# imazen/codec-eval

Measured on AMD Instinct MI355X. Metric: metric MP/s (SSIMULACRA2+DSSIM+Butteraugli) at 1/2/4/8 GPU; HBM-roofline %, higher is better.
Workload: dtype f32

## Files before the change

### codec-eval_amd/csrc/ce_api.cpp

```cpp
#include <algorithm>
#include <atomic>
#include <condition_variable>
#include <functional>
#include <mutex>
#include <thread>
#include <cmath>
#include <cstdlib>
#include <cstring>
#include <new>

#include "ce_internal.h"

static thread_local std::string g_err_noctx;

int ce_fail(ce_ctx *ctx, int code, const std::string &msg)
{
    if (ctx) ctx->err = msg; else g_err_noctx = msg;
    return code;
}

int ce_bad_length(ce_ctx *ctx, size_t want, size_t got)
{
    return ce_fail(ctx, CE_ERR_BAD_LENGTH, "Invalid image size: expected " + std::to_string(want) + " bytes, got " + std::to_string(got));
}

int ce_validate_pair(ce_ctx *ctx, size_t ref_len, size_t test_len, size_t w, size_t h)
{
    if (ref_len != test_len)
        return ce_fail(ctx, CE_ERR_DIM_MISMATCH, "Dimension mismatch: reference " + std::to_string(ref_len) +
                                                   " bytes, test " + std::to_string(test_len) + " bytes");
    if (ref_len != w * h * 3) return ce_bad_length(ctx, w * h * 3, ref_len);
    return CE_OK;
}

int ce_device_table(ce_ctx *ctx, const void *host, size_t bytes, const char *what, void **out)
{
    void *d = nullptr;
    CE_HIP(ctx, hipMalloc(&d, bytes));
    if (hipMemcpy(d, host, bytes, hipMemcpyHostToDevice) != hipSuccess) {
        hipFree(d);
        return ce_fail(ctx, CE_ERR_BACKEND, std::string("H2D failed (") + what + ")");
    }
    *out = d;
    return CE_OK;
}

static int check_map_readout(ce_ctx *ctx, const char *what, uint32_t stored, uint32_t first, uint32_t count, uint32_t block, uint32_t w,
                      uint32_t h, bool has_out, size_t out_floats)
{
    if (count == 0 || first > stored || count > stored - first)
        return ce_fail(ctx, CE_ERR_INVALID_ARG, std::string(what) + " pairs [" + std::to_string(first) + ", " + std::to_string((uint64_t)first + count) +
                                                 ") outside the " + std::to_string(stored) + " stored");
    if (block == 0 || block > 64 || (block & (block - 1)) != 0)
        return ce_fail(ctx, CE_ERR_INVALID_ARG, std::string(what) + " block must be 1 or a power of two up to 64");
    const size_t want = has_out ? (size_t)count * ((w + block - 1) / block) * ((h + block - 1) / block) : 0;
    if (out_floats != want)
        return ce_fail(ctx, CE_ERR_INVALID_ARG, std::string(what) + " readout needs " + std::to_string(want) + " floats, got " + std::to_string(out_floats));
    return CE_OK;
}

int ce_batch_butteraugli_diffmap(ce_batch *b, uint32_t first, uint32_t count, uint32_t block, float *out, size_t out_floats)
{
    if (!b || !out) return CE_ERR_INVALID_ARG;
    ce_ctx *ctx = b->ctx;
    if (b->ba_map_pairs == 0)
        return ce_fail(ctx, CE_ERR_INVALID_ARG, "no Butteraugli diffmaps: the last launch did not run Butteraugli with CE_FLAG_BUTTERAUGLI_DIFFMAP");
    if (int rc = check_map_readout(ctx, "diffmap", b->ba_map_pairs, first, count, block, b->w, b->h, true, out_floats)) return rc;
    CE_HIP(ctx, hipSetDevice(ctx->device));
    return ce_butteraugli_read_maps(b, first, count, block, out);
}

int ce_batch_dssim_ssim_maps(ce_batch *b, uint32_t level, uint32_t first, uint32_t count, uint32_t block, float *maps,
                             size_t maps_floats, double *ssim)
{
    if (!b || (!maps && !ssim)) return CE_ERR_INVALID_ARG;
    ce_ctx *ctx = b->ctx;
    if (b->ds_map_pairs == 0) return ce_fail(ctx, CE_ERR_INVALID_ARG, "no DSSIM SSIM maps: the last launch did not run DSSIM");
    if (level >= (uint32_t)b->ds_levels)
        return ce_fail(ctx, CE_ERR_INVALID_ARG, "DSSIM level " + std::to_string(level) + " of " + std::to_string(b->ds_levels));
    const auto &d = b->ds[level];
    if (int rc = check_map_readout(ctx, "SSIM map", b->ds_map_pairs, first, count, block, d.w, d.h, maps != nullptr, maps_floats)) return rc;
    CE_HIP(ctx, hipSetDevice(ctx->device));
    return ce_dssim_read_maps(b, level, first, count, block, maps, ssim);
}

int ce_batch_ssimulacra2_maps(ce_batch *b, uint32_t scale, uint32_t channel, uint32_t kind, uint32_t first, uint32_t count,
                              uint32_t block, float *maps, size_t maps_floats, double *norms)
{
    if (!b) return ce_fail(nullptr, CE_ERR_INVALID_ARG, "null handle");
    ce_ctx *ctx = b->ctx;
    if (!maps && !norms) return ce_fail(ctx, CE_ERR_INVALID_ARG, "SSIMULACRA2 maps readout without an output");
    if (b->s2_norm_pairs == 0)
        return ce_fail(ctx, CE_ERR_INVALID_ARG, "no SSIMULACRA2 maps or norms: the last launch did not run SSIMULACRA2");
    if (maps && b->s2_map_pairs == 0)
        return ce_fail(ctx, CE_ERR_INVALID_ARG, "no SSIMULACRA2 maps: the last launch did not run SSIMULACRA2 with CE_FLAG_SSIMULACRA2_MAPS");
    if (scale >= b->s2_scales_run)
        return ce_fail(ctx, CE_ERR_INVALID_ARG, "SSIMULACRA2 scale " + std::to_string(scale) + " of " + std::to_string(b->s2_scales_run) + " that ran");
    if (channel >= 3) return ce_fail(ctx, CE_ERR_INVALID_ARG, "SSIMULACRA2 channel " + std::to_string(channel) + " of 3");
    if (kind >= 3) return ce_fail(ctx, CE_ERR_INVALID_ARG, "SSIMULACRA2 map kind " + std::to_string(kind) + " of 3");
    const ce_scale_dims &d = b->sd[scale];
    if (int rc = check_map_readout(ctx, "SSIMULACRA2 map", maps ? b->s2_map_pairs : b->s2_norm_pairs, first, count, block, d.w, d.h,
                                   maps != nullptr, maps_floats))
        return rc;
    CE_HIP(ctx, hipSetDevice(ctx->device));
    return ce_ssim2_read_maps(b, scale, channel, kind, first, count, block, maps, norms);
}

static double psnr_from_sse(unsigned long long sse, size_t w, size_t h, double maxv = 255.0)
{
    const double pixel_count = (double)(w * h * 3);
    const double mse = (double)sse / pixel_count;
    if (mse == 0.0) return INFINITY;
    return 10.0 * std::log10(maxv * maxv / mse);
}

static int ce_deep_table(ce_ctx *ctx, uint32_t depth, int rule, const float **out)
{
    const auto key = std::make_pair(depth, rule);
    auto it = ctx->deep_tables.find(key);
    if (it == ctx->deep_tables.end()) {
        const uint32_t maxv = (1u << depth) - 1u;
        std::vector<float> host((size_t)maxv + 1);
        if (rule == 0) ce_build_srgb_table_f64(host.data(), maxv); else ce_build_srgb_table_powf(host.data(), maxv);
        void *d = nullptr;
        if (int rc = ce_device_table(ctx, host.data(), host.size() * sizeof(float), "deep sRGB table", &d)) return rc;
        it = ctx->deep_tables.emplace(key, static_cast<float *>(d)).first;
    }
    *out = it->second;
    return CE_OK;
}


int ce_prof_begin(ce_ctx *ctx, const char *name, hipStream_t stream)
{
    if (!ctx->prof_filter.empty()) {
        const char *f = ctx->prof_filter.c_str();
        if (f[0] == '=' ? std::strcmp(name, f + 1) != 0 : !std::strstr(name, f)) return -1;
    }
    int idx = -1;
    for (size_t i = 0; i < ctx->stats.size(); i++)
        if (ctx->stats[i].name == name) { idx = (int)i; break; }
    if (idx < 0) {
        ctx->stats.push_back(ce_kernel_stat{name, 0, 0.0});
        idx = (int)ctx->stats.size() - 1;
    }
    ce_ctx::pending pd{idx, nullptr, nullptr};
    for (hipEvent_t *e : {&pd.e0, &pd.e1}) {
        if (!ctx->event_pool.empty()) {
            *e = ctx->event_pool.back();
            ctx->event_pool.pop_back();
        } else if (hipEventCreate(e) != hipSuccess) {
            return -1;
        }
    }
    hipEventRecord(pd.e0, stream);
    ctx->pend.push_back(pd);
    return (int)ctx->pend.size() - 1;
}

void ce_prof_end(ce_ctx *ctx, int token, hipStream_t stream) { hipEventRecord(ctx->pend[token].e1, stream); }

static void prof_drain(ce_ctx *ctx)
{
    if (ctx->pend.empty()) return;
    hipSetDevice(ctx->device);
    hipStreamSynchronize(ctx->stream);
    for (auto &pd : ctx->pend) {
        float ms = 0.f;
        if (hipEventElapsedTime(&ms, pd.e0, pd.e1) == hipSuccess) {
            ctx->stats[pd.stat].launches++;
            ctx->stats[pd.stat].total_ms += ms;
        }
        ctx->event_pool.push_back(pd.e0);
        ctx->event_pool.push_back(pd.e1);
    }
    ctx->pend.clear();
}

int ce_build_xcd_list(ce_batch *b, uint32_t n_pairs, const ce_xcd_keys &keys, ce_xcd_list *L)
{
    static_assert(sizeof(ce_plan_entry) == sizeof(uint2) && alignof(ce_plan_entry) <= alignof(uint2), "entries are read as uint2");
    if (L->d && L->version == b->pair_ref_version && L->pairs == n_pairs && L->keys == keys) return CE_OK;
    ce_ctx *ctx = b->ctx;
    const std::vector<ce_plan_entry> flat = ce_plan_xcd_list(b->h_pair_ref.data(), n_pairs, b->max_refs, keys);
    if (flat.size() > L->cap) {
        if (L->d) CE_HIP(ctx, hipFree(L->d));
        L->d = nullptr;
        L->cap = 0;
        CE_HIP(ctx, hipMalloc(&L->d, flat.size() * sizeof(uint2)));
        L->cap = (uint32_t)flat.size();
    }
    if (int rc = ce_upload_table(b, L->d, flat.data(), flat.size() * sizeof(uint2))) return rc;
    L->len = (uint32_t)flat.size();
    L->version = b->pair_ref_version;
    L->pairs = n_pairs;
    L->keys = keys;
    return CE_OK;
}

void ce_free_xcd_list(ce_xcd_list *L)
{
    hipFree(L->d);
    *L = ce_xcd_list{};
}

thread_local hipStream_t ce_tls_stream = nullptr;

int ce_upload_table(ce_batch *b, void *dst, const void *src, size_t bytes)
{
    ce_ctx *ctx = b->ctx;
    if (bytes == 0) return CE_OK;
    CE_HIP(ctx, hipStreamWaitEvent(b->up_stream, b->ev_run, 0));
    CE_HIP(ctx, hipMemcpyAsync(dst, src, bytes, hipMemcpyHostToDevice, b->up_stream));
    CE_HIP(ctx, hipStreamSynchronize(b->up_stream));
    return CE_OK;
}

hipStream_t ce_ctx_aux_stream(ce_ctx *ctx, int which)
{
    if (which < 0 || which >= ce_ctx::AUX_COUNT) return nullptr;
    if (!ctx->aux_stream[which]) {
        const hipError_t e = hipStreamCreateWithFlags(&ctx->aux_stream[which], hipStreamNonBlocking);
        if (e != hipSuccess) {
            ctx->aux_stream[which] = nullptr;
            ctx->err = std::string("hipStreamCreateWithFlags (auxiliary stream): ") + hipGetErrorString(e);
        }
    }
    return ctx->aux_stream[which];
}

void ce_drain_batch(ce_batch *b)
{
    hipStreamSynchronize(b->up_stream);
    if (b->ctx->up2_stream) hipStreamSynchronize(b->ctx->up2_stream);
    hipStreamSynchronize(b->ctx->stream);
}

static void *table_of(float *p) { return p; }
static void *table_of(const ce_resample_axis &a) { return a.d; }
template <class Map>
static void free_tables(Map &m)
{
    for (auto &kv : m) hipFree(table_of(kv.second));
    m.clear();
}

static bool hdr_depth_ok(uint32_t d) { return d == 10 || d == 12 || d == 16; }

int ce_hdr_params_check(ce_ctx *ctx, uint32_t depth, float white_nits)
{
    if (!hdr_depth_ok(depth)) return ce_fail(ctx, CE_ERR_INVALID_ARG, "HDR fidelity: depth must be 10, 12 or 16, got " + std::to_string(depth));
    if (!(white_nits > 0.0f && std::isfinite(white_nits))) return ce_fail(ctx, CE_ERR_INVALID_ARG, "HDR fidelity: white_nits must be finite and > 0");
    return CE_OK;
}

extern "C" {

const char *ce_version(void) { return "codec-eval_amd 0.3.0 (gfx950)"; }

int ce_device_count(void)
{
    int n = 0;
    if (hipGetDeviceCount(&n) != hipSuccess) return -1;
    return n;
}

int ce_ctx_create_on_stream(int device, void *hip_stream, ce_ctx **out)
{
    if (!out) return CE_ERR_INVALID_ARG;
    *out = nullptr;
    int n = 0;
    if (hipGetDeviceCount(&n) != hipSuccess || n <= 0)
        return ce_fail(nullptr, CE_ERR_BACKEND, "no HIP device visible");
    if (device < 0 || device >= n) return ce_fail(nullptr, CE_ERR_INVALID_ARG, "device index out of range");
    ce_ctx *ctx = new (std::nothrow) ce_ctx();
    if (!ctx) return CE_ERR_BACKEND;
    ctx->device = device;
    auto bail = [&](const char *what, hipError_t e) {
        g_err_noctx = std::string(what) + ": " + hipGetErrorString(e);
        delete ctx;
        return CE_ERR_BACKEND;
    };
    hipError_t e;
    if ((e = hipSetDevice(device)) != hipSuccess) return bail("hipSetDevice", e);
    if (hip_stream) {
        ctx->stream = (hipStream_t)hip_stream;
        ctx->own_stream = false;
    } else {
        if ((e = hipStreamCreateWithFlags(&ctx->stream, hipStreamNonBlocking)) != hipSuccess)
            return bail("hipStreamCreate", e);
    }
    float lut[256];
    if ((e = hipMalloc(&ctx->d_lut_ssim2, sizeof(lut))) != hipSuccess) return bail("hipMalloc", e);
    if ((e = hipMalloc(&ctx->d_lut_powf, sizeof(lut))) != hipSuccess) return bail("hipMalloc", e);
    ce_build_srgb_lut_f64(lut);
    if ((e = hipMemcpy(ctx->d_lut_ssim2, lut, sizeof(lut), hipMemcpyHostToDevice)) != hipSuccess)
        return bail("hipMemcpy", e);
    ce_build_srgb_lut_powf(lut);
    if ((e = hipMemcpy(ctx->d_lut_powf, lut, sizeof(lut), hipMemcpyHostToDevice)) != hipSuccess)
        return bail("hipMemcpy", e);
    float thresh[256];
    if (!ce_build_xyb_srgb_thresholds(thresh)) {
        g_err_noctx = "host powf is not monotone around an sRGB code boundary; cannot build the XYB table";
        delete ctx;
        return CE_ERR_BACKEND;
    }
    if ((e = hipMalloc(&ctx->d_xyb_thresh, sizeof(thresh))) != hipSuccess) return bail("hipMalloc", e);
    if ((e = hipMemcpy(ctx->d_xyb_thresh, thresh, sizeof(thresh), hipMemcpyHostToDevice)) != hipSuccess)
        return bail("hipMemcpy", e);
    if ((e = hipEventCreate(&ctx->t0)) != hipSuccess) return bail("hipEventCreate", e);
    if ((e = hipEventCreate(&ctx->t1)) != hipSuccess) return bail("hipEventCreate", e);
    *out = ctx;
    return CE_OK;
}

int ce_ctx_create(int device, ce_ctx **out) { return ce_ctx_create_on_stream(device, nullptr, out); }

struct ce_fork_helpers {
    struct worker {
        std::thread th;
        std::mutex m;
        std::condition_variable cv;
        std::function<void()> job;
        bool has_job = false, done = true, stop = false;
    } w[2];
    explicit ce_fork_helpers(int device)
    {
        try {
            for (auto &x : w)
                x.th = std::thread([&x, device] {
                    (void)hipSetDevice(device);
                    std::unique_lock<std::mutex> lk(x.m);
                    for (;;) {
                        x.cv.wait(lk, [&] { return x.has_job || x.stop; });
                        if (x.stop) return;
                        x.has_job = false;
                        lk.unlock();
                        x.job();
                        lk.lock();
                        x.done = true;
                        x.cv.notify_all();
                    }
                });
        } catch (...) {
            stop_all();
            throw;
        }
    }
    void submit(int i, std::function<void()> f)
    {
        std::lock_guard<std::mutex> lk(w[i].m);
        w[i].job = std::move(f);
        w[i].has_job = true;
        w[i].done = false;
        w[i].cv.notify_all();
    }
    void wait(int i)
    {
        std::unique_lock<std::mutex> lk(w[i].m);
        w[i].cv.wait(lk, [&] { return w[i].done; });
    }
    ~ce_fork_helpers() { stop_all(); }
    void stop_all()
    {
        for (auto &x : w) {
            {
                std::lock_guard<std::mutex> lk(x.m);
                x.stop = true;
                x.cv.notify_all();
            }
            if (x.th.joinable()) x.th.join();
        }
    }
};

void ce_ctx_destroy(ce_ctx *ctx)
{
    if (!ctx) return;
    hipSetDevice(ctx->device);
    hipStreamSynchronize(ctx->stream);
    delete ctx->helpers;
    ctx->helpers = nullptr;

    prof_drain(ctx);
    for (auto &kv : ctx->shape_pool) ce_batch_destroy(kv.second);
    ctx->shape_pool.clear();
    for (ce_batch *&b : ctx->leaf_batch) ce_batch_destroy(b), b = nullptr;
    free_tables(ctx->deep_tables);
    free_tables(ctx->cicp_tables);
    free_tables(ctx->hdr_tables);
    free_tables(ctx->icc_thresholds);
    free_tables(ctx->alpha_tables);
    if (ctx->up2_stream) hipStreamSynchronize(ctx->up2_stream), hipStreamDestroy(ctx->up2_stream), hipEventDestroy(ctx->ev_up2);
    for (auto &st : ctx->aux_stream)
        if (st) hipStreamSynchronize(st), hipStreamDestroy(st), st = nullptr;
    for (hipEvent_t ev : ctx->event_pool) hipEventDestroy(ev);
    if (ctx->t0) hipEventDestroy(ctx->t0);
    if (ctx->t1) hipEventDestroy(ctx->t1);
    hipFree(ctx->leaf_d_in);
    hipFree(ctx->leaf_d_out);
    if (ctx->leaf_h) hipHostFree(ctx->leaf_h);
    hipFree(ctx->heur_d);
    if (ctx->heur_h) hipHostFree(ctx->heur_h);
    hipFree(ctx->rs_mid);
    free_tables(ctx->rs_tables);
    hipFree(ctx->d_lut_ssim2);
    hipFree(ctx->d_lut_powf);
    hipFree(ctx->d_xyb_thresh);
    if (ctx->own_stream && ctx->stream) hipStreamDestroy(ctx->stream);
    delete ctx;
}

int ce_ctx_synchronize(ce_ctx *ctx)
{
    if (!ctx) return CE_ERR_INVALID_ARG;
    CE_HIP(ctx, hipSetDevice(ctx->device));
    CE_HIP(ctx, hipStreamSynchronize(ctx->stream));
    return CE_OK;
}

void *ce_ctx_stream(ce_ctx *ctx) { return ctx ? (void *)ctx->stream : nullptr; }

static std::atomic<int> g_in_flight[64];
static std::atomic<int> &in_flight_of(const ce_ctx *ctx) { return g_in_flight[(unsigned)ctx->device % 64u]; }
static void leave_flight(ce_batch *b)
{
    if (b->counted_in_flight) {
        in_flight_of(b->ctx).fetch_sub(1, std::memory_order_relaxed);
        b->counted_in_flight = false;
    }
}

const char *ce_last_error(const ce_ctx *ctx) { return ctx ? ctx->err.c_str() : g_err_noctx.c_str(); }


static int batch_create(ce_ctx *ctx, uint32_t width, uint32_t height, uint32_t max_refs, uint32_t max_pairs, uint32_t ref_depth,
                        uint32_t test_depth, ce_batch **out, bool linear = false)
{
    if (!ctx || !out || width == 0 || height == 0 || max_refs == 0 || max_pairs == 0) return CE_ERR_INVALID_ARG;
    *out = nullptr;
    CE_HIP(ctx, hipSetDevice(ctx->device));
    const float *deep_lut[2][2] = {};
    if (ref_depth)
        for (int rule = 0; rule < 2; rule++)
            for (int side = 0; side < 2; side++)
                if (int rc = ce_deep_table(ctx, side ? test_depth : ref_depth, rule, &deep_lut[rule][side])) return rc;
    ce_batch *b = new (std::nothrow) ce_batch();
    if (!b) return CE_ERR_BACKEND;
    b->ctx = ctx;
    b->w = width;
    b->h = height;
    b->max_refs = max_refs;
    b->max_pairs = max_pairs;
    b->img_bytes = (size_t)width * height * (linear ? 12 : ref_depth ? 6 : 3);
    b->linear = linear;
    b->depth[0] = ref_depth, b->depth[1] = test_depth;
    std::memcpy(b->deep_lut, deep_lut, sizeof(deep_lut));
    b->h_pair_ref.assign(max_pairs, 0);
    static const bool keep_reference_state = [] { const char *e = std::getenv("CE_KEEP_REFERENCE_STATE"); return !(e && e[0] == '0'); }();
    b->refs.keep = keep_reference_state;
    int rc = CE_OK;
    auto chk = [&](hipError_t e, const char *what) {
        if (e != hipSuccess && rc == CE_OK) {
            ctx->err = std::string(what) + ": " + hipGetErrorString(e);
            rc = CE_ERR_BACKEND;
        }
    };
    chk(hipMalloc(&b->d_refs, b->img_bytes * max_refs + 16), "hipMalloc refs");
    chk(hipMalloc(&b->d_tests, b->img_bytes * max_pairs + 16), "hipMalloc tests");
    chk(hipMalloc(&b->d_pair_ref, sizeof(uint32_t) * (3 * (size_t)max_pairs + max_refs + 1)), "hipMalloc pair_ref");
    b->d_pair_first = b->d_pair_ref ? b->d_pair_ref + max_pairs : nullptr;
    b->d_ref_off = b->d_pair_ref ? b->d_pair_ref + 2 * (size_t)max_pairs : nullptr;
    b->d_ref_idx = b->d_pair_ref ? b->d_ref_off + max_refs + 1 : nullptr;
    chk(hipMalloc(&b->d_scores, sizeof(ce_dev_scores) * max_pairs), "hipMalloc scores");
    chk(hipHostMalloc(&b->h_scores, sizeof(ce_dev_scores) * max_pairs, hipHostMallocDefault), "hipHostMalloc scores");
    chk(hipStreamCreateWithFlags(&b->up_stream, hipStreamNonBlocking), "hipStreamCreate upload");
    chk(hipEventCreateWithFlags(&b->ev_up, hipEventDisableTiming), "hipEventCreate");
    chk(hipEventCreateWithFlags(&b->ev_run, hipEventDisableTiming), "hipEventCreate");
    for (int k = 0; k < ce_batch::kStages; k++) {
        chk(hipHostMalloc(&b->h_stage[k], b->img_bytes, hipHostMallocDefault), "hipHostMalloc stage");
        chk(hipEventCreateWithFlags(&b->ev_stage[k], hipEventDisableTiming), "hipEventCreate stage");
    }
    if (rc == CE_OK) chk(hipMemsetAsync(b->d_scores, 0, sizeof(ce_dev_scores) * max_pairs, ctx->stream), "memset");
    if (rc != CE_OK) {
        ce_batch_destroy(b);
        return rc;
    }
    *out = b;
    return CE_OK;
}

int ce_batch_create(ce_ctx *ctx, uint32_t width, uint32_t height, uint32_t max_refs, uint32_t max_pairs, ce_batch **out)
{
    return batch_create(ctx, width, height, max_refs, max_pairs, 0, 0, out);
}

int ce_batch_create_deep(ce_ctx *ctx, uint32_t width, uint32_t height, uint32_t max_refs, uint32_t max_pairs, uint32_t ref_depth,
                         uint32_t test_depth, ce_batch **out)
{
    if (!ctx || !out) return CE_ERR_INVALID_ARG;
    *out = nullptr;
    if (!ce_deep_depth_ok(ref_depth) || !ce_deep_depth_ok(test_depth))
        return ce_fail(ctx, CE_ERR_INVALID_ARG, "a deep batch's depths must be 8, 10, 12 or 16 bits, got " + std::to_string(ref_depth) +
                                                 " / " + std::to_string(test_depth));
    return batch_create(ctx, width, height, max_refs, max_pairs, ref_depth, test_depth, out);
}

int ce_batch_create_linear(ce_ctx *ctx, uint32_t width, uint32_t height, uint32_t max_refs, uint32_t max_pairs, ce_batch **out)
{
    return batch_create(ctx, width, height, max_refs, max_pairs, 0, 0, out, true);
}

void ce_batch_destroy(ce_batch *b)
{
    if (!b) return;
    hipSetDevice(b->ctx->device);
    hipStreamSynchronize(b->ctx->stream);
    leave_flight(b);
    if (b->up_stream) hipStreamSynchronize(b->up_stream), hipStreamDestroy(b->up_stream);
    for (int k = 0; k < 2; k++) {
        if (b->h_wide[k]) hipHostFree(b->h_wide[k]);
        hipFree(b->d_wide[k]);
        if (b->h_side[k]) hipHostFree(b->h_side[k]);
        hipFree(b->d_side[k]);
        if (b->ev_wide[k]) hipEventDestroy(b->ev_wide[k]);
    }
    if (b->ev_up) hipEventDestroy(b->ev_up);
    if (b->ev_run) hipEventDestroy(b->ev_run);
    if (b->ev_fork) hipEventDestroy(b->ev_fork);
    hipFree(b->d_refs);
    hipFree(b->d_refs_rt);
    hipFree(b->d_tests);
    hipFree(b->d_pair_ref);
    hipFree(b->d_scores);
    if (b->h_scores) hipHostFree(b->h_scores);
    hipFree(b->d_hdr);
    if (b->h_hdr) hipHostFree(b->h_hdr);
    hipFree(b->d_itp_map);
    hipFree(b->d_itp_over);
    if (b->h_itp_over) hipHostFree(b->h_itp_over);
    for (int k = 0; k < ce_batch::kStages; k++) {
        if (b->h_stage[k]) hipHostFree(b->h_stage[k]);
        if (b->ev_stage[k]) hipEventDestroy(b->ev_stage[k]);
    }
    for (int l = 0; l < 3; l++) {
        if (b->metric_stream[l]) hipStreamSynchronize(b->metric_stream[l]);
        if (b->ev_join[l]) hipEventDestroy(b->ev_join[l]);
    }
    ce_ssim2_free(b);
    ce_dssim_free(b);
    ce_butteraugli_free(b);
    delete b;
}

static int sync_pair_ref(ce_batch *b)
{
    if (!b->pair_ref_dirty) return CE_OK;
    const size_t P = b->max_pairs, R = b->max_refs;
    std::vector<uint32_t> table(3 * P + R + 1), first_of(R, ~0u), count(R + 1, 0);
    for (uint32_t i = 0; i < P; i++) {
        const uint32_t r = b->h_pair_ref[i];
        if (first_of[r] == ~0u) first_of[r] = i;
        table[i] = r;
        table[P + i] = first_of[r];
        count[r + 1]++;
    }
    for (size_t r = 0; r < R; r++) count[r + 1] += count[r];
    for (size_t r = 0; r <= R; r++) table[2 * P + r] = count[r];
    std::vector<uint32_t> fill(count.begin(), count.end() - 1);
    for (uint32_t i = 0; i < P; i++) table[2 * P + R + 1 + fill[b->h_pair_ref[i]]++] = i;
    if (int rc = ce_upload_table(b, b->d_pair_ref, table.data(), sizeof(uint32_t) * table.size())) return rc;
    b->pair_ref_dirty = false;
    return CE_OK;
}

int ce_batch_launch(ce_batch *b, uint32_t n_pairs, uint32_t metric_mask, uint32_t flags, float intensity_target)
{
    if (!b) return CE_ERR_INVALID_ARG;
    ce_ctx *ctx = b->ctx;
    if (n_pairs == 0 || n_pairs > b->max_pairs) return ce_fail(ctx, CE_ERR_INVALID_ARG, "n_pairs out of range");
    if (metric_mask & ~ce_known_metrics) return ce_fail(ctx, CE_ERR_INVALID_ARG, "unknown metric bit");
    if (b->depth[0] && (flags & CE_FLAG_XYB_ROUNDTRIP))
        return ce_fail(ctx, CE_ERR_INVALID_ARG, "CE_FLAG_XYB_ROUNDTRIP quantises to 8 bits by definition: not for a deep batch");
    if (b->linear && (flags & CE_FLAG_XYB_ROUNDTRIP))
        return ce_fail(ctx, CE_ERR_INVALID_ARG, "CE_FLAG_XYB_ROUNDTRIP quantises to 8 bits by definition: not for a linear batch");
    b->ba_map_pairs = b->ds_map_pairs = 0;
    b->s2_map_pairs = b->s2_norm_pairs = 0;
    CE_HIP(ctx, hipSetDevice(ctx->device));
    {
        int rc = ce_flush_uploads(b);
        if (rc != CE_OK) return rc;
    }
    if (int rc = sync_pair_ref(b)) return rc;
    uint32_t n_refs_used = 0;
    for (uint32_t i = 0; i < n_pairs; i++) n_refs_used = std::max(n_refs_used, b->h_pair_ref[i] + 1);

    const uint8_t *d_refs = b->d_refs;
    if (flags & CE_FLAG_XYB_ROUNDTRIP) {
        if (!b->d_refs_rt) CE_HIP(ctx, hipMalloc(&b->d_refs_rt, b->img_bytes * b->max_refs + 16));
        if (!b->refs.reuse(CE_REF_ROUNDTRIP, b->d_refs, n_refs_used, 0)) {
            int rc = ce_launch_xyb_roundtrip(ctx, b->d_refs, b->d_refs_rt, (size_t)n_refs_used * b->w * b->h);
            if (rc != CE_OK) return rc;
            b->refs.built(CE_REF_ROUNDTRIP, b->d_refs, n_refs_used, 0);
        }
        d_refs = b->d_refs_rt;
    }
    const bool run_ssim2 = (metric_mask & CE_METRIC_SSIMULACRA2) && b->w >= 8 && b->h >= 8;
    const bool run_dssim = (metric_mask & CE_METRIC_DSSIM) != 0;
    const bool run_ba = (metric_mask & CE_METRIC_BUTTERAUGLI) && b->w >= 8 && b->h >= 8;
    const bool store_maps = run_ba && (flags & CE_FLAG_BUTTERAUGLI_DIFFMAP);
    const bool store_ssim2_maps = run_ssim2 && (flags & CE_FLAG_SSIMULACRA2_MAPS);
    static const int fork_mask_env = [] {
        const char *e = std::getenv("CE_METRIC_STREAMS");
        if (!e || std::strcmp(e, "auto") == 0) return -1;
        if (std::strncmp(e, "fork", 4) != 0) return 0;
        if (e[4] != ':') return 7;
        int m = 0;
        if (std::strstr(e + 5, "ssim2")) m |= 1;
        if (std::strstr(e + 5, "dssim")) m |= 2;
        if (std::strstr(e + 5, "ba")) m |= 4;
        return m;
    }();
    static const double fork_below_mp = [] {
        const char *e = std::getenv("CE_METRIC_FORK_BELOW_MP");
        return e ? std::atof(e) : CE_DEFAULT_FORK_BELOW_MP;
    }();
    static const double fork_alone_below_mp = [] {
        const char *e = std::getenv("CE_METRIC_FORK_ALONE_BELOW_MP");
        return e ? std::atof(e) : CE_DEFAULT_FORK_ALONE_BELOW_MP;
    }();
    const double batch_mp = (double)n_pairs * b->w * b->h * 1e-6;
    const int others = in_flight_of(ctx).load(std::memory_order_relaxed) - (b->counted_in_flight ? 1 : 0);
    const bool by_size = batch_mp <= fork_below_mp || (others <= 0 && batch_mp <= fork_alone_below_mp);
    const unsigned fork_wanted = fork_mask_env >= 0 ? (unsigned)fork_mask_env : (by_size ? 7u : 0u);
    const unsigned fork_mask = (!ctx->prof_serial && (int)run_ssim2 + (int)run_dssim + (int)run_ba > 1) ? fork_wanted : 0u;
    hipStream_t base = ctx->stream;
    if (fork_mask) {
        if (!b->ev_fork) CE_HIP(ctx, hipEventCreateWithFlags(&b->ev_fork, hipEventDisableTiming));
        CE_HIP(ctx, hipEventRecord(b->ev_fork, base));
    }
    unsigned joined = 0;
    auto prepare_fork = [&](int k) -> int {
        if (!b->metric_stream[k]) {
            if (!(b->metric_stream[k] = ce_ctx_aux_stream(ctx, ce_ctx::AUX_METRIC0 + k))) return CE_ERR_BACKEND;
            CE_HIP(ctx, hipEventCreateWithFlags(&b->ev_join[k], hipEventDisableTiming));
        }
        CE_HIP(ctx, hipStreamWaitEvent(b->metric_stream[k], b->ev_fork, 0));
        return CE_OK;
    };
    auto launch_metric = [&](int k) -> int {
        return k == 0   ? ce_launch_ssim2(b, d_refs, n_refs_used, n_pairs, store_ssim2_maps)
               : k == 1 ? ce_launch_dssim(b, d_refs, n_refs_used, n_pairs)
                        : ce_launch_butteraugli(b, d_refs, n_refs_used, n_pairs, intensity_target, store_maps);
    };
    const bool runs[3] = {run_ssim2, run_dssim, run_ba};
    static const bool fork_threads = [] { const char *e = std::getenv("CE_FORK_THREADS"); return !(e && e[0] == '0'); }();
    if (fork_mask == 7u && fork_threads && !ctx->prof) {
        int rcs[3] = {CE_OK, CE_OK, CE_OK};
        std::string errs[3];
        int last = -1;
        for (int k = 0; k < 3; k++)
            if (runs[k]) {
                int rc = prepare_fork(k);
                if (rc != CE_OK) return rc;
                last = k;
            }
        auto body = [&](int k) {
            ce_tls_stream = b->metric_stream[k];
            rcs[k] = launch_metric(k);
            ce_tls_stream = nullptr;
            if (rcs[k] == CE_OK && hipEventRecord(b->ev_join[k], b->metric_stream[k]) != hipSuccess) rcs[k] = CE_ERR_BACKEND;
        };
        if (!ctx->helpers) {
            try {
                ctx->helpers = new ce_fork_helpers(ctx->device);
            } catch (...) {
                ctx->helpers = nullptr;
            }
        }
        int used = 0;
        for (int k = 0; k < 3; k++) {
            if (!runs[k] || k == last) continue;
            if (ctx->helpers && used < 2)
                ctx->helpers->submit(used++, [&body, k] { body(k); });
            else
                body(k);
        }
        body(last);
        for (int i = 0; i < used; i++) ctx->helpers->wait(i);
        for (int k = 0; k < 3; k++) {
            if (!runs[k]) continue;
            if (rcs[k] != CE_OK) return rcs[k];
            joined |= 1u << k;
        }
    } else {
        for (int k = 0; k < 3; k++) {
            if (!runs[k]) continue;
            if (!(fork_mask & (1u << k))) {
                int rc = launch_metric(k);
                if (rc != CE_OK) return rc;
                continue;
            }
            int rc = prepare_fork(k);
            if (rc != CE_OK) return rc;
            ce_tls_stream = b->metric_stream[k];
            rc = launch_metric(k);
            ce_tls_stream = nullptr;
            if (rc != CE_OK) return rc;
            CE_HIP(ctx, hipEventRecord(b->ev_join[k], b->metric_stream[k]));
            joined |= 1u << k;
        }
    }
    if ((metric_mask & CE_METRIC_PSNR) && b->depth[0] == b->depth[1] && !b->linear) {
        int rc = ce_launch_psnr(b, d_refs, n_pairs);
        if (rc != CE_OK) return rc;
    }
    for (int k = 0; k < 3; k++)
        if (joined & (1u << k)) CE_HIP(ctx, hipStreamWaitEvent(base, b->ev_join[k], 0));
    b->last_n_pairs = n_pairs;
    b->last_mask = metric_mask;
    b->ba_map_pairs = store_maps ? n_pairs : 0;
    b->ds_map_pairs = run_dssim ? n_pairs : 0;
    b->s2_norm_pairs = run_ssim2 ? n_pairs : 0;
    b->s2_map_pairs = store_ssim2_maps ? n_pairs : 0;
    b->s2_scales_run = run_ssim2 ? (uint32_t)std::min(b->n_scales, b->debug_max_scales) : 0;
    CE_HIP(ctx, hipMemcpyAsync(b->h_scores, b->d_scores, sizeof(ce_dev_scores) * n_pairs, hipMemcpyDeviceToHost, ctx->stream));
    CE_HIP(ctx, hipEventRecord(b->ev_run, ctx->stream));
    b->run_pending = true;
    b->inline_pending = false;
    if (!b->counted_in_flight) {
        in_flight_of(ctx).fetch_add(1, std::memory_order_relaxed);
        b->counted_in_flight = true;
    }
    return CE_OK;
}

int ce_batch_collect(ce_batch *b, uint32_t n_pairs, ce_scores *out)
{
    if (!b || !out) return CE_ERR_INVALID_ARG;
    ce_ctx *ctx = b->ctx;
    if (n_pairs == 0 || n_pairs > b->max_pairs) return ce_fail(ctx, CE_ERR_INVALID_ARG, "n_pairs out of range");
    CE_HIP(ctx, hipSetDevice(ctx->device));
    if (n_pairs > b->last_n_pairs) return ce_fail(ctx, CE_ERR_INVALID_ARG, "collect asks for more pairs than the last launch ran");
    CE_HIP(ctx, hipEventSynchronize(b->ev_run));
    b->run_pending = false;
    leave_flight(b);
    const uint32_t mask = b->last_mask;
    for (uint32_t i = 0; i < n_pairs; i++) {
        ce_scores s{};
        s.status = CE_OK;
        const ce_dev_scores &d = b->h_scores[i];
        if ((mask & CE_METRIC_PSNR) && b->depth[0] == b->depth[1] && !b->linear) {
            s.psnr = psnr_from_sse(d.sse, b->w, b->h, b->depth[0] ? (double)((1u << b->depth[0]) - 1u) : 255.0);
            s.valid |= CE_METRIC_PSNR;
        }
        if (mask & CE_METRIC_DSSIM) {
            s.dssim = d.dssim;
            s.valid |= CE_METRIC_DSSIM;
        }
        if (mask & CE_METRIC_BUTTERAUGLI) {
            if (b->w < 8 || b->h < 8) {
                s.status = CE_ERR_TOO_SMALL;
            } else {
                s.butteraugli = d.butteraugli;
                s.valid |= CE_METRIC_BUTTERAUGLI;
            }
        }
        if (mask & CE_METRIC_SSIMULACRA2) {
            if (b->w < 8 || b->h < 8) {
                s.status = CE_ERR_TOO_SMALL;
            } else {
                s.ssimulacra2 = d.ssimulacra2;
                s.valid |= CE_METRIC_SSIMULACRA2;
            }
        }
        out[i] = s;
    }
    return CE_OK;
}

int ce_batch_butteraugli_pnorm3(ce_batch *b, uint32_t n_pairs, double *out)
{
    if (!b || !out || !b->ba_ready || n_pairs == 0 || n_pairs > b->max_pairs) return CE_ERR_INVALID_ARG;
    ce_ctx *ctx = b->ctx;
    CE_HIP(ctx, hipSetDevice(ctx->device));
    CE_HIP(ctx, hipStreamSynchronize(ctx->stream));
    CE_HIP(ctx, hipMemcpy(out, b->ba_pnorm, sizeof(double) * n_pairs, hipMemcpyDeviceToHost));
    return CE_OK;
}

int ce_batch_run(ce_batch *b, uint32_t n_pairs, uint32_t metric_mask, uint32_t flags, float intensity_target,
                 ce_scores *out)
{
    if (int rc = ce_batch_launch(b, n_pairs, metric_mask, flags, intensity_target)) return rc;
    return ce_batch_collect(b, n_pairs, out);
}


size_t ce_estimate_batch_bytes(uint32_t w, uint32_t h, uint32_t n_refs, uint32_t n_pairs, uint32_t metric_mask)
{
    const double px = (double)w * h, slots = (double)n_refs + n_pairs, pairs = n_pairs;
    double bytes = 3.0 * px * slots + 64.0 * pairs;
    double allocations = 8;
    if (metric_mask & CE_METRIC_SSIMULACRA2) {
        bytes += px * (20.0 * slots + 80.0 * pairs);
        allocations += 24;
    }
    if (metric_mask & CE_METRIC_DSSIM) {
        bytes += px * (6.0 * slots + 48.0 * n_refs + 17.4 * pairs);
        allocations += 24;
    }
    if (metric_mask & CE_METRIC_BUTTERAUGLI) {
        bytes += px * (91.0 * slots + 10.0 * n_refs + 1.0 * pairs);
        allocations += 20;
    }
    if (metric_mask & CE_METRIC_PSNR) bytes += 8.0 * pairs;
    return (size_t)(bytes * 1.2) + (size_t)(allocations * (256u << 10)) + (8u << 20);
}

size_t ce_estimate_batch_bytes_deep(uint32_t w, uint32_t h, uint32_t n_refs, uint32_t n_pairs, uint32_t metric_mask, uint32_t ref_depth,
                                    uint32_t test_depth)
{
    if (!ce_deep_depth_ok(ref_depth) || !ce_deep_depth_ok(test_depth)) return 0;
    const size_t slabs = (size_t)3 * w * h * ((size_t)n_refs + n_pairs);
    return ce_estimate_batch_bytes(w, h, n_refs, n_pairs, metric_mask) + slabs + (((size_t)8 << ref_depth) + ((size_t)8 << test_depth));
}

size_t ce_estimate_batch_bytes_linear(uint32_t w, uint32_t h, uint32_t n_refs, uint32_t n_pairs, uint32_t metric_mask)
{
    return ce_estimate_batch_bytes(w, h, n_refs, n_pairs, metric_mask) + (size_t)9 * w * h * ((size_t)n_refs + n_pairs);
}

int ce_ctx_memory_info(ce_ctx *ctx, size_t *free_bytes, size_t *total_bytes)
{
    if (!ctx || !free_bytes || !total_bytes) return CE_ERR_INVALID_ARG;
    CE_HIP(ctx, hipSetDevice(ctx->device));
    CE_HIP(ctx, hipMemGetInfo(free_bytes, total_bytes));
    return CE_OK;
}

int ce_host_alloc(ce_ctx *ctx, size_t bytes, void **out)
{
    if (!ctx || !out || bytes == 0) return CE_ERR_INVALID_ARG;
    *out = nullptr;
    CE_HIP(ctx, hipSetDevice(ctx->device));
    CE_HIP(ctx, hipHostMalloc(out, bytes, hipHostMallocDefault));
    return CE_OK;
}

int ce_host_free(ce_ctx *ctx, void *p)
{
    if (!p) return CE_OK;
    const hipError_t e = hipHostFree(p);
    if (e != hipSuccess) {
        if (ctx) ctx->err = std::string("hipHostFree: ") + hipGetErrorString(e);
        return CE_ERR_BACKEND;
    }
    return CE_OK;
}

static size_t chunk_budget(ce_ctx *ctx)
{
    if (const char *e = std::getenv("CE_EVAL_BATCH_BYTES")) {
        const long long v = std::atoll(e);
        if (v > 0) return (size_t)v;
    }
    size_t free_b = 0, total_b = 0;
    if (hipMemGetInfo(&free_b, &total_b) != hipSuccess) return (size_t)8 << 30;
    size_t pooled = 0;
    for (auto &kv : ctx->shape_pool) {
        const ce_batch *pb = kv.second;
        const uint32_t held = (pb->ssim2_ready ? CE_METRIC_SSIMULACRA2 : 0u) | (pb->dssim_ready ? CE_METRIC_DSSIM : 0u) |
                              (pb->ba_ready ? CE_METRIC_BUTTERAUGLI : 0u);
        pooled += ce_estimate_batch_bytes(pb->w, pb->h, pb->max_refs, pb->max_pairs, held);
    }
    const size_t share = (size_t)((double)(free_b + pooled) * 0.8 / ce_ctx::kPoolRing);
    return std::min(share, ce_ctx::kChunkBytesMax);
}

static void pool_evict_idle(ce_ctx *ctx)
{
    for (auto it = ctx->shape_pool.begin(); it != ctx->shape_pool.end();) {
        if (!it->second->run_pending && !it->second->uploads_pending) {
            ce_batch_destroy(it->second);
            it = ctx->shape_pool.erase(it);
        } else {
            ++it;
        }
    }
}

static int shape_batch(ce_ctx *ctx, uint32_t w, uint32_t h, uint32_t need_pairs, uint32_t ring_slot, ce_batch **out)
{
    auto key = std::make_tuple(w, h, ring_slot);
    auto it = ctx->shape_pool.find(key);
    if (it != ctx->shape_pool.end() && it->second->max_pairs >= need_pairs) {
        *out = it->second;
        return CE_OK;
    }
    if (it != ctx->shape_pool.end()) {
        ce_batch_destroy(it->second);
        ctx->shape_pool.erase(it);
    }
    ce_batch *b = nullptr;
    int rc = ce_batch_create(ctx, w, h, need_pairs, need_pairs, &b);
    if (rc == CE_ERR_BACKEND) {
        pool_evict_idle(ctx);
        rc = ce_batch_create(ctx, w, h, need_pairs, need_pairs, &b);
    }
    if (rc != CE_OK) return rc;
    ctx->shape_pool[key] = b;
    *out = b;
    return CE_OK;
}

int ce_eval_batch(ce_ctx *ctx, size_t n, const ce_pair_desc *pairs, uint32_t metric_mask, uint32_t flags,
                  float intensity_target, ce_scores *out)
{
    return ce_eval_batch_lut(ctx, n, pairs, nullptr, metric_mask, flags, intensity_target, out);
}

int ce_eval_batch_lut(ce_ctx *ctx, size_t n, const ce_pair_desc *pairs, const ce_lut *const *test_luts, uint32_t metric_mask,
                      uint32_t flags, float intensity_target, ce_scores *out)
{
    if (!ctx || (!pairs && n) || (!out && n)) return CE_ERR_INVALID_ARG;
    if (flags & CE_FLAG_BUTTERAUGLI_DIFFMAP)
        return ce_fail(ctx, CE_ERR_INVALID_ARG, "CE_FLAG_BUTTERAUGLI_DIFFMAP needs a ce_batch or a ce_ref: the pooled batches keep no maps");
    if (flags & CE_FLAG_SSIMULACRA2_MAPS)
        return ce_fail(ctx, CE_ERR_INVALID_ARG, "CE_FLAG_SSIMULACRA2_MAPS needs a ce_batch or a ce_ref: the pooled batches keep no maps");
    std::map<std::pair<uint32_t, uint32_t>, std::vector<size_t>> buckets;
    for (size_t i = 0; i < n; i++) {
        out[i] = ce_scores{};
        const ce_pair_desc &d = pairs[i];
        int rc = (!d.reference || !d.test || d.width == 0 || d.height == 0)
                     ? CE_ERR_INVALID_ARG
                     : ce_validate_pair(ctx, d.reference_len, d.test_len, d.width, d.height);
        if (rc != CE_OK) {
            out[i].status = rc;
            continue;
        }
        if (test_luts && test_luts[i] && test_luts[i]->ctx->device != ctx->device)
            return ce_fail(ctx, CE_ERR_INVALID_ARG, "colour table and batch are on different devices");
        buckets[{d.width, d.height}].push_back(i);
    }
    if (buckets.empty()) return CE_OK;
    if (metric_mask & ~ce_known_metrics) return ce_fail(ctx, CE_ERR_INVALID_ARG, "unknown metric bit");
    static const size_t forced_chunks = [] {
        const char *e = std::getenv("CE_EVAL_BATCH_CHUNKS");
        const int v = e ? std::atoi(e) : 0;
        return (size_t)(v >= 1 && v <= (int)ce_ctx::kPoolRing ? v : 0);
    }();
    static const size_t ramp0 = [] {
        const char *e = std::getenv("CE_EVAL_BATCH_RAMP");
        return (size_t)(e ? std::max(0, std::atoi(e)) : 64);
    }();
    std::vector<ce_plan_chunk> plan;
    struct launched { ce_batch *b = nullptr; std::vector<size_t> items; };
    std::vector<launched> running;
    ce_batch *filling = nullptr;
    int rc = CE_OK;
    auto collect = [&](size_t c) -> int {
        const launched l = std::exchange(running[c], launched{});
        std::vector<ce_scores> tmp(l.items.size());
        const int r = ce_batch_collect(l.b, (uint32_t)tmp.size(), tmp.data());
        for (size_t k = 0; k < tmp.size() && r == CE_OK && rc == CE_OK; k++) out[l.items[k]] = tmp[k];
        return r;
    };
    auto run_chunk = [&](uint32_t w, uint32_t h, size_t c) -> int {
        const ce_plan_chunk &p = plan[c];
        if (p.collect_first != ce_plan_none)
            if (int r = collect(p.collect_first)) return r;
        ce_batch *b = nullptr;
        if (int r = shape_batch(ctx, w, h, p.max_pairs, p.slot, &b)) return r;
        filling = b;
        std::vector<ce_upload_job> jobs;
        std::vector<size_t> items;
        for (uint32_t s = 0; s < p.refs.size(); s++) {
            jobs.push_back({b->d_refs + (size_t)s * b->img_bytes, pairs[p.refs[s][0]].reference});
            for (size_t i : p.refs[s]) {
                if (int r = ce_batch_bind_pair(b, (uint32_t)items.size(), s)) return r;
                jobs.push_back({b->d_tests + items.size() * b->img_bytes, pairs[i].test});
                items.push_back(i);
            }
        }
        ce_invalidate_reference_state(b);
        if (int r = ce_upload_many(b, jobs)) return r;
        if (test_luts)
            for (size_t k = 0; k < items.size(); k++)
                if (int r = ce_apply_lut(b, b->d_tests + k * b->img_bytes, test_luts[items[k]])) return r;
        if (int r = ce_batch_launch(b, (uint32_t)items.size(), metric_mask, flags, intensity_target)) return r;
        running[c] = {b, std::move(items)};
        return CE_OK;
    };
    uint32_t ring = 0;
    for (auto it = buckets.begin(); it != buckets.end() && rc == CE_OK; ++it) {
        const uint32_t w = it->first.first, h = it->first.second;
        std::vector<const void *> refs;
        for (size_t i : it->second) refs.push_back(pairs[i].reference);
        const size_t per_pair = ce_estimate_batch_bytes(w, h, 1, 2, metric_mask) - ce_estimate_batch_bytes(w, h, 1, 1, metric_mask) +
                                ce_estimate_batch_bytes(w, h, 2, 1, metric_mask) - ce_estimate_batch_bytes(w, h, 1, 1, metric_mask);
        auto pooled = ctx->shape_pool.find(std::make_tuple(w, h, 0u));
        const ce_plan_inputs in{chunk_budget(ctx), per_pair, pooled != ctx->shape_pool.end() ? pooled->second->max_pairs : 0u, forced_chunks, ramp0};
        const size_t first = plan.size();
        ce_plan_bucket(it->second, refs, in, ring, plan);
        running.resize(plan.size());
        for (size_t c = first; c < plan.size() && rc == CE_OK; c++) rc = run_chunk(w, h, c);
    }
    for (size_t c = 0; c < plan.size(); c++)
        if (running[c].b) {
            const int r = collect(c);
            if (rc == CE_OK) rc = r;
        }
    if (rc != CE_OK && filling) ce_drain_batch(filling);
    return rc;
}


int ce_batch_image_heuristics(ce_batch *b, uint32_t which, uint32_t first, uint32_t count, ce_image_heuristics *out)
{
    if (!b || !out) return CE_ERR_INVALID_ARG;
    ce_ctx *ctx = b->ctx;
    if (b->depth[0]) return ce_fail(ctx, CE_ERR_INVALID_ARG, "image heuristics are defined on u8 gray levels: not for a deep batch");
    if (b->linear) return ce_fail(ctx, CE_ERR_INVALID_ARG, "image heuristics are defined on u8 gray levels: not for a linear batch");
    if (which != CE_BATCH_REFERENCES && which != CE_BATCH_TESTS)
        return ce_fail(ctx, CE_ERR_INVALID_ARG, "image heuristics: unknown slab " + std::to_string(which));
    const uint32_t slots = which == CE_BATCH_TESTS ? b->max_pairs : b->max_refs;
    if (count == 0 || first > slots || count > slots - first)
        return ce_fail(ctx, CE_ERR_INVALID_ARG, "image heuristics: images [" + std::to_string(first) + ", " +
                                                 std::to_string((uint64_t)first + count) + ") outside the " + std::to_string(slots) +
                                                 " slots");
    if (b->w < 3 || b->h < 3)
        return ce_fail(ctx, CE_ERR_TOO_SMALL, "image heuristics need at least 3 x 3 pixels, got " + std::to_string(b->w) + " x " +
                                               std::to_string(b->h));
    CE_HIP(ctx, hipSetDevice(ctx->device));
    if (int rc = ce_flush_uploads(b)) return rc;
    const uint8_t *slab = which == CE_BATCH_TESTS ? b->d_tests : b->d_refs;
    return ce_image_heuristics_run(ctx, slab + (size_t)first * b->img_bytes, b->img_bytes, b->w, b->h, count, out);
}


int ce_pq_code_thresholds(uint32_t depth, float white_nits, float *out, size_t n)
{
    if (!out || !hdr_depth_ok(depth) || n != ((size_t)1 << depth) - 1)
        return ce_fail(nullptr, CE_ERR_INVALID_ARG, "ce_pq_code_thresholds: depth 10, 12 or 16 and n = 2^depth - 1");
    if (!ce_build_pq_code_thresholds((1u << depth) - 1u, (double)white_nits, out))
        return ce_fail(nullptr, CE_ERR_INVALID_ARG, "ce_pq_code_thresholds: white_nits must be finite and > 0");
    return CE_OK;
}

int ce_hdr_fidelity_matrices(float a[9], float b[9])
{
    if (!a || !b) return ce_fail(nullptr, CE_ERR_INVALID_ARG, "ce_hdr_fidelity_matrices: null pointer");
    ce_build_hdr_fidelity_matrices(a, b);
    return CE_OK;
}

static int hdr_table_dev(ce_ctx *ctx, uint32_t depth, float white_nits, const float **table, const float **coarse)
{
    uint32_t white_bits;
    std::memcpy(&white_bits, &white_nits, 4);
    const size_t n = ((size_t)1 << depth) - 1, padded = (n + 15) & ~(size_t)15, n_coarse = depth > 12 ? ((size_t)1 << 12) - 1 : 0;
    const auto key = std::make_pair(depth, white_bits);
    auto it = ctx->hdr_tables.find(key);
    if (it == ctx->hdr_tables.end()) {
        std::vector<float> host(padded + n_coarse, INFINITY);
        ce_build_pq_code_thresholds((uint32_t)n, (double)white_nits, host.data());
        const size_t stride = (size_t)1 << (depth > 12 ? depth - 12 : 0);
        for (size_t j = 0; j < n_coarse; j++) host[padded + j] = host[(j + 1) * stride - 1];
        void *d = nullptr;
        if (int rc = ce_device_table(ctx, host.data(), host.size() * sizeof(float), "PQ code thresholds", &d)) return rc;
        it = ctx->hdr_tables.emplace(key, static_cast<float *>(d)).first;
    }
    *table = it->second;
    *coarse = n_coarse ? it->second + padded : it->second;
    return CE_OK;
}

int ce_batch_hdr_fidelity(ce_batch *b, uint32_t n_pairs, uint32_t depth, float white_nits, ce_hdr_scores *out)
{
    if (!b) return CE_ERR_INVALID_ARG;
    ce_ctx *ctx = b->ctx;
    if (!out) return ce_fail(ctx, CE_ERR_INVALID_ARG, "HDR fidelity: null pointer");
    if (!b->linear)
        return ce_fail(ctx, CE_ERR_INVALID_ARG, "HDR fidelity reads linear light: it needs a linear batch (ce_batch_create_linear)");
    if (int rc = ce_hdr_params_check(ctx, depth, white_nits)) return rc;
    if (n_pairs == 0 || n_pairs > b->max_pairs) return ce_fail(ctx, CE_ERR_INVALID_ARG, "n_pairs out of range");
    CE_HIP(ctx, hipSetDevice(ctx->device));
    const float *d_table = nullptr, *d_coarse = nullptr;
    if (int rc = hdr_table_dev(ctx, depth, white_nits, &d_table, &d_coarse)) return rc;
    if (!b->d_hdr) CE_HIP(ctx, hipMalloc(&b->d_hdr, sizeof(unsigned long long) * 3 * b->max_pairs));
    if (!b->h_hdr) CE_HIP(ctx, hipHostMalloc(&b->h_hdr, sizeof(unsigned long long) * 3 * b->max_pairs, hipHostMallocDefault));
    if (int rc = ce_flush_uploads(b)) return rc;
    if (int rc = sync_pair_ref(b)) return rc;
    float a[9], lms[9];
    ce_build_hdr_fidelity_matrices(a, lms);
    if (int rc = ce_launch_hdr_fidelity(b, n_pairs, depth, d_table, d_coarse, a, lms, b->d_hdr)) return rc;
    CE_HIP(ctx, hipMemcpyAsync(b->h_hdr, b->d_hdr, sizeof(unsigned long long) * 3 * n_pairs, hipMemcpyDeviceToHost, ctx->stream));
    CE_HIP(ctx, hipStreamSynchronize(ctx->stream));
    const double maxv = (double)((1u << depth) - 1u), n_px = (double)((size_t)b->w * b->h);
    for (uint32_t i = 0; i < n_pairs; i++) {
        ce_hdr_scores s{};
        s.pq_sse = b->h_hdr[3 * i], s.itp_sum_q20 = b->h_hdr[3 * i + 1], s.itp_max_q20 = b->h_hdr[3 * i + 2];
        s.pq_psnr = psnr_from_sse(s.pq_sse, b->w, b->h, maxv);
        s.delta_e_itp_mean = (double)s.itp_sum_q20 / 1048576.0 / n_px;
        s.delta_e_itp_max = (double)s.itp_max_q20 / 1048576.0;
        out[i] = s;
    }
    return CE_OK;
}

int ce_batch_delta_e_itp_map(ce_batch *b, uint32_t first, uint32_t count, uint32_t depth, float white_nits, uint32_t block, uint32_t *map,
                             size_t map_len, const uint32_t *thresholds_q20, uint32_t n_thresholds, uint64_t *over)
{
    if (!b) return ce_fail(nullptr, CE_ERR_INVALID_ARG, "Delta E ITP map: null batch");
    ce_ctx *ctx = b->ctx;
    if (!b->linear)
        return ce_fail(ctx, CE_ERR_INVALID_ARG, "the Delta E ITP map reads linear light: it needs a linear batch (ce_batch_create_linear)");
    if (int rc = ce_hdr_params_check(ctx, depth, white_nits)) return rc;
    if (!map && !over) return ce_fail(ctx, CE_ERR_INVALID_ARG, "Delta E ITP map: neither a map nor counts asked for");
    if (count == 0 || first > b->max_pairs || count > b->max_pairs - first)
        return ce_fail(ctx, CE_ERR_INVALID_ARG, "Delta E ITP map: pairs [" + std::to_string(first) + ", " + std::to_string((uint64_t)first + count) +
                                                 ") outside the batch's " + std::to_string(b->max_pairs));
    if (int rc = check_map_readout(ctx, "Delta E ITP map", b->max_pairs, first, count, block, b->w, b->h, map != nullptr, map_len)) return rc;
    if (n_thresholds > CE_DELTA_E_ITP_MAX_THRESHOLDS)
        return ce_fail(ctx, CE_ERR_INVALID_ARG, "Delta E ITP map: at most " + std::to_string(CE_DELTA_E_ITP_MAX_THRESHOLDS) + " thresholds, got " +
                                                 std::to_string(n_thresholds));
    if (over && (n_thresholds == 0 || !thresholds_q20)) return ce_fail(ctx, CE_ERR_INVALID_ARG, "Delta E ITP map: counts asked for without thresholds");
    if (!over && (n_thresholds != 0 || thresholds_q20)) return ce_fail(ctx, CE_ERR_INVALID_ARG, "Delta E ITP map: thresholds given without a place for the counts");
    CE_HIP(ctx, hipSetDevice(ctx->device));
    const float *d_table = nullptr, *d_coarse = nullptr;
    if (int rc = hdr_table_dev(ctx, depth, white_nits, &d_table, &d_coarse)) return rc;
    if (map && b->itp_map_cap < map_len) {
        hipFree(b->d_itp_map);
        b->d_itp_map = nullptr, b->itp_map_cap = 0;
        CE_HIP(ctx, hipMalloc(&b->d_itp_map, map_len * sizeof(uint32_t)));
        b->itp_map_cap = map_len;
    }
    const size_t over_bytes = sizeof(unsigned long long) * CE_DELTA_E_ITP_MAX_THRESHOLDS;
    if (over && !b->d_itp_over) CE_HIP(ctx, hipMalloc(&b->d_itp_over, over_bytes * b->max_pairs));
    if (over && !b->h_itp_over) CE_HIP(ctx, hipHostMalloc(&b->h_itp_over, over_bytes * b->max_pairs, hipHostMallocDefault));
    if (int rc = ce_flush_uploads(b)) return rc;
    if (int rc = sync_pair_ref(b)) return rc;
    float a[9], lms[9];
    ce_build_hdr_fidelity_matrices(a, lms);
    if (int rc = ce_launch_delta_e_itp_map(b, first, count, depth, d_table, d_coarse, a, lms, block, map ? b->d_itp_map : nullptr, thresholds_q20,
                                           n_thresholds, over ? b->d_itp_over : nullptr))
        return rc;
    if (map) CE_HIP(ctx, hipMemcpyAsync(map, b->d_itp_map, map_len * sizeof(uint32_t), hipMemcpyDeviceToHost, ctx->stream));
    if (over) CE_HIP(ctx, hipMemcpyAsync(b->h_itp_over, b->d_itp_over, over_bytes * count, hipMemcpyDeviceToHost, ctx->stream));
    CE_HIP(ctx, hipStreamSynchronize(ctx->stream));
    for (uint32_t i = 0; over && i < count; i++)
        for (uint32_t j = 0; j < n_thresholds; j++) over[(size_t)i * n_thresholds + j] = b->h_itp_over[(size_t)i * CE_DELTA_E_ITP_MAX_THRESHOLDS + j];
    return CE_OK;
}


struct ce_ref {
    ce_ctx *ctx;
    ce_batch *batch;
    uint32_t flags;
};

int ce_ref_create(ce_ctx *ctx, const uint8_t *reference, size_t reference_len, uint32_t width, uint32_t height,
                  uint32_t flags, ce_ref **out)
{
    if (!ctx || !reference || !out) return CE_ERR_INVALID_ARG;
    *out = nullptr;
    if (reference_len != (size_t)width * height * 3) return ce_bad_length(ctx, (size_t)width * height * 3, reference_len);
    ce_batch *b = nullptr;
    int rc = ce_batch_create(ctx, width, height, 1, 1, &b);
    if (rc != CE_OK) return rc;
    rc = ce_batch_set_reference(b, 0, reference, reference_len);
    if (rc != CE_OK) {
        ce_batch_destroy(b);
        return rc;
    }
    b->refs.keep = true;
    *out = new ce_ref{ctx, b, flags};
    return CE_OK;
}

int ce_ref_compare_many(ce_ref *ref, const uint8_t *const *tests, const size_t *test_lens, uint32_t n_tests,
                        uint32_t metric_mask, float intensity_target, ce_scores *out)
{
    if (!ref || !tests || !test_lens || !out) return CE_ERR_INVALID_ARG;
    if (n_tests == 0) return CE_OK;
    ce_ctx *ctx = ref->ctx;
    ce_batch *b = ref->batch;
    CE_HIP(ctx, hipSetDevice(ctx->device));
    if (n_tests > b->max_pairs) {
        ce_batch *nb = nullptr;
        int rc = ce_batch_create(ctx, b->w, b->h, 1, n_tests, &nb);
        if (rc != CE_OK) return rc;
        rc = ce_flush_uploads(b);
        if (rc != CE_OK) return rc;
        CE_HIP(ctx, hipMemcpyAsync(nb->d_refs, b->d_refs, b->img_bytes, hipMemcpyDeviceToDevice, ctx->stream));
        CE_HIP(ctx, hipStreamSynchronize(ctx->stream));
        ce_invalidate_reference_state(nb);
        nb->refs.keep = true;
        for (int k = 0; k < 3; k++) nb->refs.builds[k] = b->refs.builds[k];
        ce_batch_destroy(b);
        ref->batch = b = nb;
    }
    bool any_ok = false;
    for (uint32_t i = 0; i < n_tests; i++) {
        out[i] = ce_scores{};
        if (!tests[i]) return CE_ERR_INVALID_ARG;
        if (test_lens[i] != b->img_bytes) {
            out[i].status = ce_fail(ctx, CE_ERR_DIM_MISMATCH, "Dimension mismatch: reference " + std::to_string(b->img_bytes) +
                                                               " bytes, test " + std::to_string(test_lens[i]) + " bytes");
            continue;
        }
        any_ok = true;
    }
    if (!any_ok) return CE_OK;
    std::vector<ce_scores> tmp(n_tests);
    b->caller_blocks = true;
    int rc = CE_OK;
    for (uint32_t i = 0; i < n_tests && rc == CE_OK; i++)
        rc = out[i].status != CE_OK ? ce_batch_bind_pair(b, i, 0) : ce_batch_set_test(b, i, 0, tests[i], test_lens[i]);
    if (rc == CE_OK) rc = ce_batch_run(b, n_tests, metric_mask, ref->flags, intensity_target, tmp.data());
    if (rc != CE_OK) ce_drain_batch(b);
    b->caller_blocks = false;
    if (rc != CE_OK) return rc;
    for (uint32_t i = 0; i < n_tests; i++)
        if (out[i].status == CE_OK) out[i] = tmp[i];
    return CE_OK;
}

int ce_ref_compare(ce_ref *ref, const uint8_t *test, size_t test_len, uint32_t metric_mask, float intensity_target,
                   ce_scores *out)
{
    if (!ref || !test || !out) return CE_ERR_INVALID_ARG;
    int rc = ce_ref_compare_many(ref, &test, &test_len, 1, metric_mask, intensity_target, out);
    if (rc != CE_OK) return rc;
    return out->status;
}

int ce_ref_butteraugli_diffmap(ce_ref *ref, uint32_t first, uint32_t count, uint32_t block, float *out, size_t out_floats)
{
    if (!ref) return CE_ERR_INVALID_ARG;
    return ce_batch_butteraugli_diffmap(ref->batch, first, count, block, out, out_floats);
}

int ce_ref_dssim_ssim_maps(ce_ref *ref, uint32_t level, uint32_t first, uint32_t count, uint32_t block, float *maps,
                           size_t maps_floats, double *ssim)
{
    if (!ref) return CE_ERR_INVALID_ARG;
    return ce_batch_dssim_ssim_maps(ref->batch, level, first, count, block, maps, maps_floats, ssim);
}

int ce_ref_ssimulacra2_maps(ce_ref *ref, uint32_t scale, uint32_t channel, uint32_t kind, uint32_t first, uint32_t count, uint32_t block,
                            float *maps, size_t maps_floats, double *norms)
{
    if (!ref) return ce_fail(nullptr, CE_ERR_INVALID_ARG, "null handle");
    return ce_batch_ssimulacra2_maps(ref->batch, scale, channel, kind, first, count, block, maps, maps_floats, norms);
}

int ce_ref_image_heuristics(ce_ref *ref, ce_image_heuristics *out)
{
    if (!ref || !out) return CE_ERR_INVALID_ARG;
    return ce_batch_image_heuristics(ref->batch, CE_BATCH_REFERENCES, 0, 1, out);
}

int ce_ssimulacra2_scales(uint32_t width, uint32_t height, uint32_t *n_scales, uint32_t *scale_w, uint32_t *scale_h)
{
    if (!n_scales || !scale_w || !scale_h) return ce_fail(nullptr, CE_ERR_INVALID_ARG, "null pointer");
    if (width == 0 || height == 0) return ce_fail(nullptr, CE_ERR_INVALID_ARG, "empty image");
    *n_scales = ce_plan_ssim2_scales(width, height, CE_SSIM2_MAX_SCALES, scale_w, scale_h);
    return CE_OK;
}

int ce_dssim_levels(uint32_t width, uint32_t height, uint32_t *n_levels, uint32_t *level_w, uint32_t *level_h)
{
    if (!n_levels || !level_w || !level_h) return ce_fail(nullptr, CE_ERR_INVALID_ARG, "null pointer");
    if (width == 0 || height == 0) return ce_fail(nullptr, CE_ERR_INVALID_ARG, "empty image");
    *n_levels = ce_plan_dssim_levels(width, height, CE_DSSIM_MAX_LEVELS, level_w, level_h);
    return CE_OK;
}

int ce_ref_stats(const ce_ref *ref, uint32_t builds[3])
{
    if (!ref || !builds) return CE_ERR_INVALID_ARG;
    return ce_batch_ref_stats(ref->batch, builds);
}

int ce_batch_ref_stats(const ce_batch *b, uint32_t builds[3])
{
    if (!b || !builds) return CE_ERR_INVALID_ARG;
    for (int k = 0; k < 3; k++) builds[k] = b->refs.builds[k];
    return CE_OK;
}

void ce_ref_destroy(ce_ref *ref)
{
    if (!ref) return;
    ce_batch_destroy(ref->batch);
    delete ref;
}


int ce_prof_enable(ce_ctx *ctx, int on)
{
    if (!ctx) return CE_ERR_INVALID_ARG;
    prof_drain(ctx);
    ctx->prof = on != 0;
    ctx->prof_serial = on == 1;
    return CE_OK;
}

int ce_prof_filter(ce_ctx *ctx, const char *substring)
{
    if (!ctx) return CE_ERR_INVALID_ARG;
    prof_drain(ctx);
    ctx->prof_filter = substring ? substring : "";
    return CE_OK;
}

int ce_prof_reset(ce_ctx *ctx)
{
    if (!ctx) return CE_ERR_INVALID_ARG;
    prof_drain(ctx);
    ctx->stats.clear();
    return CE_OK;
}

int ce_prof_count(ce_ctx *ctx)
{
    if (!ctx) return 0;
    prof_drain(ctx);
    return (int)ctx->stats.size();
}

int ce_prof_get(ce_ctx *ctx, int index, const char **name, uint64_t *launches, double *total_ms)
{
    if (!ctx || index < 0 || index >= (int)ctx->stats.size()) return CE_ERR_INVALID_ARG;
    prof_drain(ctx);
    if (name) *name = ctx->stats[index].name.c_str();
    if (launches) *launches = ctx->stats[index].launches;
    if (total_ms) *total_ms = ctx->stats[index].total_ms;
    return CE_OK;
}

int ce_timer_start(ce_ctx *ctx)
{
    if (!ctx) return CE_ERR_INVALID_ARG;
    CE_HIP(ctx, hipSetDevice(ctx->device));
    CE_HIP(ctx, hipEventRecord(ctx->t0, ctx->stream));
    return CE_OK;
}

int ce_timer_stop(ce_ctx *ctx, double *elapsed_ms)
{
    if (!ctx || !elapsed_ms) return CE_ERR_INVALID_ARG;
    CE_HIP(ctx, hipSetDevice(ctx->device));
    CE_HIP(ctx, hipEventRecord(ctx->t1, ctx->stream));
    CE_HIP(ctx, hipEventSynchronize(ctx->t1));
    float ms = 0.f;
    CE_HIP(ctx, hipEventElapsedTime(&ms, ctx->t0, ctx->t1));
    *elapsed_ms = ms;
    return CE_OK;
}


int ce_debug_ssim2_planes(ce_batch *b, int scale, int which, int channel, float *out, size_t out_floats,
                          uint32_t *w_out, uint32_t *h_out)
{
    if (!b || !out || !b->ssim2_ready || scale < 0 || scale >= b->n_scales) return CE_ERR_INVALID_ARG;
    ce_ctx *ctx = b->ctx;
    const ce_scale_dims &d = b->sd[scale];
    const int nplanes = which == 4 ? CE_SSIM2_STREAMS : 3;
    if (out_floats < (size_t)nplanes * d.w * d.h) return CE_ERR_INVALID_ARG;
    const uint32_t ref_slot = b->h_pair_ref[0], test_slot = b->max_refs;
    const float *src = nullptr;
    switch (which) {
        case 0:
        case 1:
            if (scale == 0) return CE_ERR_INVALID_ARG;
            src = b->d_lin[scale] + (size_t)(which == 0 ? ref_slot : test_slot) * 3 * d.plane;
            break;
        case 2: src = b->d_xyb[scale] + (size_t)ref_slot * 3 * d.plane; break;
        case 3: src = b->d_xyb[scale] + (size_t)test_slot * 3 * d.plane; break;
        case 4:
            if (channel < 0 || channel > 2) return CE_ERR_INVALID_ARG;
            src = b->d_hbuf[scale] + (size_t)channel * CE_SSIM2_STREAMS * d.hplane;
            break;
        default: return CE_ERR_INVALID_ARG;
    }
    CE_HIP(ctx, hipSetDevice(ctx->device));
    CE_HIP(ctx, hipStreamSynchronize(ctx->stream));
    const size_t spl = which == 4 ? d.hplane : d.plane, spitch = which == 4 ? d.hpitch : d.pitch;
    for (int p = 0; p < nplanes; p++)
        CE_HIP(ctx, hipMemcpy2D(out + (size_t)p * d.w * d.h, (size_t)d.w * sizeof(float), src + (size_t)p * spl,
                                spitch * sizeof(float), (size_t)d.w * sizeof(float), d.h, hipMemcpyDeviceToHost));
    if (w_out) *w_out = d.w;
    if (h_out) *h_out = d.h;
    return CE_OK;
}

int ce_debug_ssim2_limit_scales(ce_batch *b, int max_scales)
{
    if (!b || max_scales < 1 || max_scales > CE_MAX_SCALES) return CE_ERR_INVALID_ARG;
    b->debug_max_scales = max_scales;
    return CE_OK;
}

int ce_debug_dssim_walk_rows(ce_batch *b, uint32_t rows)
{
    if (!b || (rows != 0 && (rows < 2 || rows > 64 || (rows & (rows - 1)) != 0))) return CE_ERR_INVALID_ARG;
    b->debug_ds_rows = rows;
    b->refs.of[CE_REF_DSSIM].invalidate();
    return CE_OK;
}

int ce_debug_ssim2_averages(ce_batch *b, uint32_t pair_index, double *avg, int *n_scales)
{
    if (!b || !avg || !b->ssim2_ready || pair_index >= b->max_pairs) return CE_ERR_INVALID_ARG;
    ce_ctx *ctx = b->ctx;
    CE_HIP(ctx, hipSetDevice(ctx->device));
    CE_HIP(ctx, hipStreamSynchronize(ctx->stream));
    CE_HIP(ctx, hipMemcpy(avg, b->d_avg + (size_t)pair_index * CE_MAX_SCALES * 18, sizeof(double) * CE_MAX_SCALES * 18,
                          hipMemcpyDeviceToHost));
    if (n_scales) *n_scales = b->n_scales;
    return CE_OK;
}

int ce_debug_ssim2_occupancy(int which) { return ce_ssim2_occupancy(which); }

int ce_debug_div_sweep(ce_ctx *ctx, uint64_t seed, uint64_t count, uint64_t *mismatches)
{
    if (!ctx || count == 0) return CE_ERR_INVALID_ARG;
    CE_HIP(ctx, hipSetDevice(ctx->device));
    return ce_butteraugli_div_sweep(ctx, seed, count, mismatches);
}

int ce_debug_calibrate_traffic(ce_ctx *ctx, size_t bytes)
{
    if (!ctx) return CE_ERR_INVALID_ARG;
    CE_HIP(ctx, hipSetDevice(ctx->device));
    return ce_calibrate_traffic(ctx, bytes);
}

int ce_debug_cbrt_sweep(ce_ctx *ctx, uint32_t first_bits, uint64_t count, uint64_t *mismatches, uint64_t *slow_path)
{
    if (!ctx || count == 0 || (uint64_t)first_bits + count > (1ull << 32)) return CE_ERR_INVALID_ARG;
    CE_HIP(ctx, hipSetDevice(ctx->device));
    return ce_ssim2_cbrt_sweep(ctx, first_bits, count, mismatches, slow_path);
}

}
```

### codec-eval_amd/csrc/ce_internal.h

```cpp
#pragma once

#include <hip/hip_runtime.h>

#include <cstdint>
#include <cstdio>
#include <functional>
#include <map>
#include <string>
#include <tuple>
#include <utility>
#include <vector>

#include "ce_metrics.h"
#include "ce_metrics_debug.h"
#include "ce_plan.h"
#include "ce_ref_state.h"

#define CE_MAX_SCALES 6
#define CE_SSIM2_STREAMS 5
#define CE_DSSIM_SCALES 5
enum { CE_SRC_F32 = 0, CE_SRC_U8 = 1, CE_SRC_U16 = 2, CE_SRC_LIN = 3 };
static_assert(CE_MAX_SCALES == CE_SSIM2_MAX_SCALES, "the ABI's scale count is the pyramid's");

struct ce_scale_dims {
    uint32_t w, h, pitch;
    size_t plane;
    uint32_t hpitch;
    size_t hplane;
};

struct ce_dev_scores {
    double dssim;
    double ssimulacra2;
    double butteraugli;
    unsigned long long sse;
};

struct ce_kernel_stat {
    std::string name;
    uint64_t launches = 0;
    double total_ms = 0.0;
};

#ifndef CE_DEFAULT_FORK_BELOW_MP
#define CE_DEFAULT_FORK_BELOW_MP 4.0
#endif
#ifndef CE_DEFAULT_FORK_ALONE_BELOW_MP
#define CE_DEFAULT_FORK_ALONE_BELOW_MP 64.0
#endif

struct ce_resample_axis {
    void *d = nullptr;
    uint32_t n_in = 0, n_out = 0, ksize = 0;
};

enum ce_leaf_kind { CE_LEAF_RGB8 = 0, CE_LEAF_DEEP = 1, CE_LEAF_LINEAR = 2, CE_LEAF_KINDS = 3 };

struct ce_ctx {
    int device = 0;
    hipStream_t stream = nullptr;
    bool own_stream = true;
    std::string err;

    float *d_lut_ssim2 = nullptr;
    float *d_lut_powf = nullptr;
    float *d_xyb_thresh = nullptr;
    std::map<std::pair<uint32_t, int>, float *> deep_tables;
    struct ce_batch *leaf_batch[CE_LEAF_KINDS] = {};
    std::map<std::tuple<int, uint32_t, uint32_t>, float *> cicp_tables;
    std::map<std::pair<uint32_t, uint32_t>, float *> hdr_tables;
    std::map<uint32_t, float *> icc_thresholds;
    std::map<uint32_t, float *> alpha_tables;

    bool prof = false;
    bool prof_serial = false;
    std::string prof_filter;
    std::vector<ce_kernel_stat> stats;
    struct pending { int stat; hipEvent_t e0, e1; };
    std::vector<pending> pend;
    std::vector<hipEvent_t> event_pool;
    hipEvent_t t0 = nullptr, t1 = nullptr;

    static constexpr uint32_t kPoolRing = ce_plan_ring_slots;
    static constexpr size_t kChunkBytesMax = (size_t)48 << 30;
    std::map<std::tuple<uint32_t, uint32_t, uint32_t>, ce_batch *> shape_pool;

    uint8_t *leaf_d_in = nullptr, *leaf_d_out = nullptr, *leaf_h = nullptr;
    size_t leaf_in_cap = 0, leaf_out_cap = 0, leaf_h_cap = 0;
    uint8_t *heur_d = nullptr, *heur_h = nullptr;
    size_t heur_d_cap = 0, heur_h_cap = 0;
    uint8_t *rs_mid = nullptr;
    size_t rs_mid_cap = 0;
    std::map<std::tuple<uint32_t, uint32_t, int, bool>, ce_resample_axis> rs_tables;

    enum { AUX_METRIC0 = 0, AUX_SSIM2_L0 = 3, AUX_BA_HALF = 4, AUX_COUNT = 5 };
    hipStream_t aux_stream[AUX_COUNT] = {};
    hipStream_t up2_stream = nullptr;
    hipEvent_t ev_up2 = nullptr;

    struct ce_fork_helpers *helpers = nullptr;
};

struct ce_xcd_list {
    uint2 *d = nullptr;
    uint32_t len = 0, cap = 0, version = ~0u, pairs = 0;
    ce_xcd_keys keys{};
};

struct ce_batch {
    ce_ctx *ctx = nullptr;
    uint32_t w = 0, h = 0, max_refs = 0, max_pairs = 0;
    size_t img_bytes = 0;
    bool linear = false;
    uint32_t depth[2] = {0, 0};
    const float *deep_lut[2][2] = {};

    uint8_t *d_refs = nullptr;
    uint8_t *d_refs_rt = nullptr;
    uint8_t *d_tests = nullptr;
    uint32_t *d_pair_ref = nullptr;
    uint32_t *d_pair_first = nullptr;
    uint32_t *d_ref_off = nullptr, *d_ref_idx = nullptr;
    std::vector<uint32_t> h_pair_ref;
    bool pair_ref_dirty = true;
    uint32_t pair_ref_version = 0;
    static constexpr int kStages = 8;
    uint8_t *h_stage[kStages] = {};
    hipEvent_t ev_stage[kStages] = {};
    bool stage_busy[kStages] = {};
    int next_stage = 0;
    hipStream_t up_stream = nullptr;
    hipEvent_t ev_up = nullptr, ev_run = nullptr;
    bool uploads_pending = false, run_pending = false;
    bool inline_pending = false;
    bool counted_in_flight = false;
    uint8_t *h_wide[2] = {}, *d_wide[2] = {};
    size_t wide_cap[2] = {};
    hipEvent_t ev_wide[2] = {};
    bool wide_busy[2] = {};
    int next_wide = 0;
    uint8_t *h_side[2] = {}, *d_side[2] = {};

    int n_scales = 0;
    ce_scale_dims sd[CE_MAX_SCALES];
    float *d_lin[CE_MAX_SCALES] = {};
    float *d_xyb[CE_MAX_SCALES] = {};
    float *d_hbuf[CE_MAX_SCALES] = {};
    hipStream_t lvl_stream[CE_MAX_SCALES] = {};
    hipStream_t metric_stream[3] = {};
    hipEvent_t ev_fork = nullptr, ev_join[3] = {};
    hipEvent_t ev_prep[CE_MAX_SCALES] = {}, ev_done[CE_MAX_SCALES] = {};
    double *d_partials = nullptr;
    uint32_t max_vblocks = 0;
    double *d_avg = nullptr;
    float *s2_map = nullptr;
    float *s2_map_lvl[CE_MAX_SCALES] = {};
    uint32_t s2_map_pairs = 0, s2_norm_pairs = 0, s2_scales_run = 0;
    float *s2_cells = nullptr;
    size_t s2_cells_cap = 0;
    ce_dev_scores *d_scores = nullptr;
    ce_dev_scores *h_scores = nullptr;
    bool ssim2_ready = false;
    ce_xcd_list work_h, work_v;
    ce_xcd_list work_ht, work_vt;
    ce_ref_states refs;
    int debug_max_scales = CE_MAX_SCALES;

    struct dssim_level { uint32_t w, h, pitch; size_t plane; };
    int ds_levels = 0;
    dssim_level ds[CE_DSSIM_SCALES];
    float *ds_lin[2] = {};
    float *ds_img = nullptr;
    float *ds_rimg[CE_DSSIM_SCALES] = {}, *ds_rmu[CE_DSSIM_SCALES] = {}, *ds_rsq[CE_DSSIM_SCALES] = {};
    float *ds_map = nullptr;
    double *ds_part = nullptr;
    double *ds_level_scores = nullptr;
    uint32_t ds_map_pairs = 0;
    float *ds_cells = nullptr;
    size_t ds_cells_cap = 0;
    uint32_t ds_blocks = 0;
    uint32_t debug_ds_rows = 0;
    ce_xcd_list ds_gwork[CE_DSSIM_SCALES];
    bool dssim_ready = false;

    struct ba_level { uint32_t w, h, pitch; size_t plane; };
    ba_level ba[2];
    int ba_levels = 0;
    float *ba_psy[2] = {};
    float *ba_diff[2] = {};
    float *ba_mask[2] = {};
    float *ba_s[3] = {};
    float *ba_s_half[3] = {};
    hipStream_t ba_half_stream = nullptr;
    hipEvent_t ev_ba_fork = nullptr, ev_ba_join = nullptr;
    float *ba_mask_vals[2] = {};
    float *ba_map = nullptr;
    uint32_t ba_map_pairs = 0;
    float *ba_cells = nullptr;
    size_t ba_cells_cap = 0;
    float *ba_blk_max = nullptr;
    double *ba_blk_sums = nullptr;
    double *ba_pnorm = nullptr;
    uint32_t ba_blocks = 0;
    ce_xcd_list ba_work[2];
    bool ba_ready = false;

    unsigned long long *d_hdr = nullptr, *h_hdr = nullptr;
    uint32_t *d_itp_map = nullptr;
    size_t itp_map_cap = 0;
    unsigned long long *d_itp_over = nullptr, *h_itp_over = nullptr;

    uint32_t last_n_pairs = 0;
    bool caller_blocks = false;
    uint32_t last_mask = 0;
};

#define CE_HIP(ctx_, expr)                                                                         \
    do {                                                                                           \
        hipError_t e__ = (expr);                                                                   \
        if (e__ != hipSuccess) {                                                                   \
            (ctx_)->err = std::string(#expr) + ": " + hipGetErrorString(e__);                      \
            return CE_ERR_BACKEND;                                                                 \
        }                                                                                          \
    } while (0)


int ce_fail(ce_ctx *ctx, int code, const std::string &msg);
int ce_bad_length(ce_ctx *ctx, size_t want, size_t got);
inline bool ce_deep_depth_ok(uint32_t d) { return d == 8 || d == 10 || d == 12 || d == 16; }

struct ce_lut {
    ce_ctx *ctx;
    uint32_t *d_table;
};
struct ce_icc_lut;
struct ce_icc {
    ce_ctx *ctx;
    float m[9];
    bool has_matrix;
    float *d_tables[4];
    ce_icc_lut *lut = nullptr;
};
struct ce_icc_lut {
    bool tetra;
    float *d_clut;
    uint32_t grid[3];
    float *d_samples;
    ce_icc_lut_curve curves[6];
    float mat[12];
    bool has_matrix;
    uint32_t pcs;
};
inline int ce_icc_depth_index(uint32_t depth) { return depth == 8 ? 0 : depth == 10 ? 1 : depth == 12 ? 2 : 3; }
struct ce_upload_job {
    uint8_t *dst;
    const uint8_t *src;
};

int ce_order_write(ce_batch *b, bool on_ctx_stream);
int ce_flush_uploads(ce_batch *b);
void ce_invalidate_reference_state(ce_batch *b);
int ce_upload_many(ce_batch *b, const std::vector<ce_upload_job> &jobs);
int ce_apply_lut(ce_batch *b, uint8_t *slot, const ce_lut *lut);
int ce_leaf_scratch(ce_ctx *ctx, size_t in_bytes, size_t out_bytes);
int ce_leaf_roundtrip(ce_ctx *ctx, const void *in, size_t in_bytes, void *out, size_t out_bytes,
                      const std::function<int(uint8_t *, uint8_t *)> &launch);
int ce_leaf_roundtrip(ce_ctx *ctx, size_t in_bytes, const std::function<void(uint8_t *, uint8_t *)> &fill, void *out, size_t out_bytes,
                      const std::function<int(uint8_t *, uint8_t *)> &launch);

int ce_upload_table(ce_batch *b, void *dst, const void *src, size_t bytes);
int ce_device_table(ce_ctx *ctx, const void *host, size_t bytes, const char *what, void **out);
constexpr uint32_t ce_known_metrics = CE_METRIC_DSSIM | CE_METRIC_SSIMULACRA2 | CE_METRIC_BUTTERAUGLI | CE_METRIC_PSNR;
int ce_validate_pair(ce_ctx *ctx, size_t ref_len, size_t test_len, size_t w, size_t h);
void ce_drain_batch(ce_batch *b);
int ce_hdr_params_check(ce_ctx *ctx, uint32_t depth, float white_nits);

hipStream_t ce_ctx_aux_stream(ce_ctx *ctx, int which);

int ce_prof_begin(ce_ctx *ctx, const char *name, hipStream_t stream);
void ce_prof_end(ce_ctx *ctx, int token, hipStream_t stream);

extern thread_local hipStream_t ce_tls_stream;
#define CE_STREAM(ctx_) (ce_tls_stream ? ce_tls_stream : (ctx_)->stream)

#define CE_LAUNCH_ON(ctx_, stream_, name_, kern_, grid_, block_, shmem_, ...)                      \
    do {                                                                                           \
        int tok__ = (ctx_)->prof ? ce_prof_begin((ctx_), name_, (stream_)) : -1;                   \
        hipLaunchKernelGGL(kern_, grid_, block_, shmem_, (stream_), __VA_ARGS__);                  \
        if (tok__ >= 0) ce_prof_end((ctx_), tok__, (stream_));                                     \
    } while (0)
#define CE_LAUNCH(ctx_, name_, kern_, grid_, block_, shmem_, ...)                                  \
    CE_LAUNCH_ON(ctx_, CE_STREAM(ctx_), name_, kern_, grid_, block_, shmem_, __VA_ARGS__)

#if defined(__HIPCC__)
__device__ __forceinline__ float ce_div_refined(float a, float b, float r)
{
    float q = a * r;
    q = __builtin_fmaf(__builtin_fmaf(-b, q, a), r, q);
    return __builtin_fmaf(__builtin_fmaf(-b, q, a), r, q);
}
__device__ __forceinline__ float ce_rcp_refined(float b)
{
    const float r0 = __builtin_amdgcn_rcpf(b);
    return __builtin_fmaf(__builtin_fmaf(-b, r0, 1.0f), r0, r0);
}
__device__ __forceinline__ float ce_div_noscale(float a, float b) { return ce_div_refined(a, b, ce_rcp_refined(b)); }
#endif

int ce_launch_psnr(ce_batch *b, const uint8_t *d_refs, uint32_t n_pairs);
int ce_launch_ingest(ce_ctx *ctx, hipStream_t stream, int format, const void *d_src, uint8_t *d_dst, size_t n_pixels);
int ce_launch_ingest_deep(ce_ctx *ctx, hipStream_t stream, int format, uint32_t depth, const void *d_src, uint16_t *d_dst, size_t n_pixels);
int ce_launch_lut_expand(ce_ctx *ctx, hipStream_t stream, const uint8_t *d_packed, uint32_t *d_table);
int ce_launch_lut_apply(ce_ctx *ctx, hipStream_t stream, uint8_t *d_rgb, const uint32_t *d_table, size_t n_pixels);
int ce_ssim2_prepare(ce_batch *b);
void ce_ssim2_free(ce_batch *b);
int ce_launch_ssim2(ce_batch *b, const uint8_t *d_refs, uint32_t n_refs_used, uint32_t n_pairs, bool store_maps);
int ce_ssim2_read_maps(ce_batch *b, uint32_t scale, uint32_t channel, uint32_t kind, uint32_t first, uint32_t count,
                       uint32_t block, float *maps, double *norms);
int ce_ssim2_occupancy(int which);
int ce_ssim2_cbrt_sweep(ce_ctx *ctx, uint32_t first_bits, uint64_t count, uint64_t *mismatches, uint64_t *slow_path);
int ce_launch_xyb_roundtrip(ce_ctx *ctx, const uint8_t *d_in, uint8_t *d_out, size_t n_pixels);
int ce_launch_dssim(ce_batch *b, const uint8_t *d_refs, uint32_t n_refs_used, uint32_t n_pairs);
void ce_dssim_free(ce_batch *b);
int ce_launch_butteraugli(ce_batch *b, const uint8_t *d_refs, uint32_t n_refs_used, uint32_t n_pairs, float intensity_target,
                          bool store_map);
int ce_butteraugli_read_maps(ce_batch *b, uint32_t first, uint32_t count, uint32_t block, float *out);
int ce_dssim_read_maps(ce_batch *b, uint32_t level, uint32_t first, uint32_t count, uint32_t block, float *maps, double *ssim);
struct ce_map_geom {
    uint32_t w, h, pitch;
    size_t plane;
};
int ce_read_map_cells(ce_batch *b, const char *name, const float *map, ce_map_geom g, uint32_t first, uint32_t count, uint32_t block,
                      bool take_min, float **cells, size_t *cells_cap, float *out);
void ce_butteraugli_free(ce_batch *b);
int ce_butteraugli_div_sweep(ce_ctx *ctx, uint64_t seed, uint64_t count, uint64_t *mismatches);
int ce_calibrate_traffic(ce_ctx *ctx, size_t bytes);
int ce_build_xcd_list(ce_batch *b, uint32_t n_pairs, const ce_xcd_keys &keys, ce_xcd_list *list);
void ce_free_xcd_list(ce_xcd_list *list);
int ce_launch_rgb8_to_dssim_image(ce_ctx *ctx, const uint8_t *d_rgb, float *d_rgba, size_t n_pixels);
int ce_image_heuristics_run(ce_ctx *ctx, const uint8_t *d_imgs, size_t img_stride, uint32_t w, uint32_t h, uint32_t n,
                            ce_image_heuristics *out);

int ce_launch_resample(ce_ctx *ctx, hipStream_t stream, const uint8_t *d_src, size_t src_stride, uint8_t *d_dst, size_t dst_stride,
                       uint32_t w, uint32_t h, uint32_t out_w, uint32_t out_h, uint32_t n, const ce_resample_axis *horiz,
                       const ce_resample_axis *vert, uint8_t *mid);
inline int ce_resample_launched(ce_ctx *ctx)
{
    const hipError_t e = hipGetLastError();
    if (e == hipSuccess) return CE_OK;
    ctx->err = std::string("resample: ") + hipGetErrorString(e);
    return CE_ERR_BACKEND;
}

int ce_launch_resample_f32(ce_ctx *ctx, hipStream_t stream, const float *d_src, size_t src_stride, float *d_dst, size_t dst_stride,
                           uint32_t w, uint32_t h, uint32_t out_w, uint32_t out_h, uint32_t n, const ce_resample_axis *horiz,
                           const ce_resample_axis *vert, float *mid);

struct ce_yuv_dev {
    const uint8_t *plane[3];
    size_t pitch[3];
    int subsampling, layout, upsample;
    uint32_t depth, shift;
    int64_t k[7];
};
int ce_launch_yuv(ce_ctx *ctx, hipStream_t stream, const ce_yuv_dev &src, uint32_t w, uint32_t h, void *d_dst, bool out16, uint32_t depth_out);
template <class YuvArgs>
inline void ce_fill_yuv_args(YuvArgs &a, const ce_yuv_dev &src, uint32_t w, uint32_t h, int64_t m)
{
    a.p0 = src.plane[0], a.p1 = src.plane[1], a.p2 = src.plane[2];
    a.pitch0 = src.pitch[0], a.pitch1 = src.pitch[1], a.pitch2 = src.pitch[2];
    a.w = w, a.h = h;
    a.cw = src.subsampling == CE_YUV_444 ? w : (w + 1) / 2;
    a.ch = src.subsampling == CE_YUV_420 ? (h + 1) / 2 : h;
    a.shift = src.shift, a.maxv = (1u << src.depth) - 1u;
    a.triangle = src.upsample == CE_CHROMA_TRIANGLE;
    a.ky = src.k[0], a.krv = src.k[1], a.kgu = src.k[2], a.kgv = src.k[3], a.kbu = src.k[4], a.y0 = src.k[5], a.c0 = src.k[6];
    a.m = m;
}

int ce_launch_alpha(ce_ctx *ctx, hipStream_t stream, const void *d_src, bool src16, void *d_dst, bool dst16, uint32_t depth,
                    size_t n_pixels, uint32_t n_bg, const uint16_t *backgrounds);

struct ce_tensor_dev {
    const void *data;
    int64_t stride_n, stride_c, stride_y, stride_x;
    int dtype;
    int quantise;
};
int ce_launch_tensor(ce_ctx *ctx, hipStream_t stream, const ce_tensor_dev &src, uint32_t w, uint32_t h, uint32_t count, void *d_dst,
                     size_t slot_bytes, int slot, uint32_t depth);

int ce_launch_linear_sanitise(ce_ctx *ctx, hipStream_t stream, const float *d_src, float *d_dst, size_t n_samples);
struct ce_linear_pixel {
    const float *d_table;
    uint32_t maxv;
    bool has_matrix;
    float m[9];
    bool hlg = false;
    double hlg_params[5];
};
template <class HlgArgs>
inline void ce_fill_pixel_args(HlgArgs &a, float *d_dst, const ce_linear_pixel &px)
{
    a.c.dst = d_dst, a.c.table = px.d_table, a.c.maxv = px.maxv;
    if (px.has_matrix)
        for (int i = 0; i < 9; i++) a.c.m[i] = px.m[i];
    if (px.hlg) a.kr = px.hlg_params[0], a.kg = px.hlg_params[1], a.kb = px.hlg_params[2], a.gm1 = px.hlg_params[3], a.a = px.hlg_params[4];
}
int ce_launch_tagged(ce_ctx *ctx, hipStream_t stream, int format, const void *d_src, float *d_dst, size_t n_pixels, const ce_linear_pixel &px);
int ce_launch_yuv_tagged(ce_ctx *ctx, hipStream_t stream, const ce_yuv_dev &src, uint32_t w, uint32_t h, float *d_dst, const ce_linear_pixel &px);
struct ce_gainmap_plan {
    ce_linear_pixel base;
    uint32_t gw, gh, channels;
    double base_offset[3], alternate_offset[3];
    double ytab[3 * 256];
    size_t table_bytes() const { return (size_t)channels * 256 * sizeof(double); }
    size_t map_bytes() const { return (size_t)gw * gh * channels; }
};
int ce_launch_gainmap(ce_ctx *ctx, hipStream_t stream, int format, const void *d_src, const uint8_t *d_side, float *d_dst, uint32_t w, uint32_t h,
                      const ce_gainmap_plan &plan);

struct ce_icc_pixel {
    const float *d_tables = nullptr;
    uint32_t maxv = 0;
    bool has_matrix = false;
    float m[9] = {};
    uint32_t depth_out = 0;
    bool out16 = false;
    const float *d_thr = nullptr;
    const ce_icc_lut *lut = nullptr;
};
struct ce_over_plan;
int ce_launch_icc(ce_ctx *ctx, hipStream_t stream, int format, const void *d_src, void *d_dst, size_t n_pixels, const ce_icc_pixel &px,
                  const ce_over_plan *ov = nullptr);
int ce_launch_icc_lut(ce_ctx *ctx, hipStream_t stream, int format, const void *d_src, void *d_dst, size_t n_pixels, const ce_icc_pixel &px,
                      const ce_over_plan *ov = nullptr);
template <class IccArgs>
inline void ce_fill_icc_args(IccArgs &a, const ce_icc_pixel &px)
{
    a.c.maxv = px.maxv;
    a.c.table = px.d_tables, a.table_g = px.d_tables + (size_t)px.maxv + 1, a.table_b = px.d_tables + 2 * ((size_t)px.maxv + 1);
    if (px.has_matrix)
        for (int i = 0; i < 9; i++) a.c.m[i] = px.m[i];
}
template <class IccLutArgs>
inline void ce_fill_icc_lut_args(IccLutArgs &a, const ce_icc_pixel &px)
{
    const ce_icc_lut *lut = px.lut;
    a.c.maxv = px.maxv;
    a.c.table = px.d_tables, a.table_g = px.d_tables + (size_t)px.maxv + 1, a.table_b = px.d_tables + 2 * ((size_t)px.maxv + 1);
    for (int i = 0; i < 9; i++) a.c.m[i] = px.m[i];
    a.clut = reinterpret_cast<decltype(a.clut)>(lut->d_clut);
    if (lut->d_clut) {
        a.s0 = lut->grid[1] * lut->grid[2], a.s1 = lut->grid[2];
        a.i0 = lut->grid[0] - 2, a.i1 = lut->grid[1] - 2, a.i2 = lut->grid[2] - 2;
        a.g0 = (float)(lut->grid[0] - 1), a.g1 = (float)(lut->grid[1] - 1), a.g2 = (float)(lut->grid[2] - 1);
    }
    a.has_matrix = lut->has_matrix, a.pcs = lut->pcs;
    for (int i = 0; i < 12; i++) a.mat[i] = lut->mat[i];
    for (int k = 0; k < 6; k++) {
        const ce_icc_lut_curve &c = lut->curves[k];
        auto &o = k < 3 ? a.mc[k] : a.bc[k - 3];
        o.kind = (uint32_t)c.kind;
        o.n = c.kind == CE_ICC_LUT_CURVE_SAMPLED ? c.count : c.ftype;
        o.s = c.kind == CE_ICC_LUT_CURVE_SAMPLED ? lut->d_samples + c.first_sample : nullptr;
        for (int i = 0; i < 7; i++) o.q[i] = c.q[i];
        (k < 3 ? a.has_m : a.has_b) |= c.kind != CE_ICC_LUT_CURVE_IDENTITY;
    }
}
int ce_launch_yuv_icc(ce_ctx *ctx, hipStream_t stream, const ce_yuv_dev &src, uint32_t w, uint32_t h, void *d_dst, const ce_icc_pixel &px);
int ce_launch_yuv_icc_0(ce_ctx *ctx, hipStream_t stream, const ce_yuv_dev &src, uint32_t w, uint32_t h, void *d_dst, const ce_icc_pixel &px);
int ce_launch_yuv_icc_1(ce_ctx *ctx, hipStream_t stream, const ce_yuv_dev &src, uint32_t w, uint32_t h, void *d_dst, const ce_icc_pixel &px);
int ce_launch_yuv_icc_2(ce_ctx *ctx, hipStream_t stream, const ce_yuv_dev &src, uint32_t w, uint32_t h, void *d_dst, const ce_icc_pixel &px);

struct ce_over_plan {
    const float *d_atab = nullptr;
    uint32_t n_bg = 0;
    float bg[CE_MAX_BACKGROUNDS][3] = {};
    size_t slot_floats = 0;
};
int ce_launch_tagged_over(ce_ctx *ctx, hipStream_t stream, int format, const void *d_src, float *d_dst, size_t n_pixels, const ce_linear_pixel &px,
                          const ce_over_plan &ov);
int ce_launch_linear_over(ce_ctx *ctx, hipStream_t stream, const float *d_src, float *d_dst, size_t n_pixels, bool premultiplied,
                          const ce_over_plan &ov);
template <class OverArgs>
inline void ce_fill_over_args(OverArgs &o, const ce_over_plan &ov)
{
    o.atab = ov.d_atab, o.n_bg = ov.n_bg, o.slot_floats = ov.slot_floats;
    for (uint32_t k = 0; k < CE_MAX_BACKGROUNDS; k++)
        for (int c = 0; c < 3; c++) o.bg[k][c] = ov.bg[k][c];
}

int ce_launch_hdr_fidelity(ce_batch *b, uint32_t n_pairs, uint32_t depth, const float *d_table, const float *d_coarse, const float a[9],
                           const float lms[9], unsigned long long *d_out);

int ce_launch_delta_e_itp_map(ce_batch *b, uint32_t first, uint32_t count, uint32_t depth, const float *d_table, const float *d_coarse,
                              const float a[9], const float lms[9], uint32_t block, uint32_t *d_map, const uint32_t *thresholds,
                              uint32_t n_thresholds, unsigned long long *d_over);

bool ce_build_pq_code_thresholds(uint32_t maxv, double white_nits, float *out);
void ce_build_hdr_fidelity_matrices(float a[9], float b[9]);
void ce_build_hlg_table(uint32_t maxv, float *lut);
double ce_build_gainmap_weight(const ce_gainmap *g);
void ce_build_gainmap_tables(const ce_gainmap *g, uint32_t channels, double *out);
bool ce_build_luminance_row(int primaries, double k[3]);
bool ce_build_transfer_table(int transfer, uint32_t maxv, double white_nits, float *lut);
bool ce_build_colour_matrix(int primaries, float m[9]);
bool ce_build_resample_table(uint32_t n_in, uint32_t n_out, int filter, std::vector<int32_t> &table, uint32_t *ksize);
bool ce_build_resample_table_f64(uint32_t n_in, uint32_t n_out, int filter, std::vector<double> &table, uint32_t *ksize);
void ce_build_srgb_lut_f64(float lut[256]);
void ce_build_srgb_lut_powf(float lut[256]);
void ce_build_srgb_table_f64(float *lut, uint32_t maxv);
void ce_build_srgb_table_powf(float *lut, uint32_t maxv);
void ce_ssim2_recursive_gaussian(float mul_in[3], float mul_prev[3]);
bool ce_build_xyb_srgb_thresholds(float thresh[256]);
```

### codec-eval_amd/csrc/ce_plan.h

```cpp
#pragma once

#include <algorithm>
#include <cstdint>
#include <map>
#include <vector>

inline constexpr uint32_t ce_plan_ring_slots = 3;
inline constexpr size_t ce_plan_none = ~(size_t)0;

struct ce_plan_inputs {
    size_t budget;
    size_t per_pair;
    uint32_t pooled_pairs;
    size_t forced_chunks;
    size_t ramp;
};

struct ce_plan_chunk {
    uint32_t slot;
    uint32_t max_pairs;
    size_t collect_first;
    std::vector<std::vector<size_t>> refs;
};

inline void ce_plan_bucket(const std::vector<size_t> &items, const std::vector<const void *> &refs, const ce_plan_inputs &in,
                           uint32_t &ring, std::vector<ce_plan_chunk> &plan)
{
    std::map<const void *, size_t> group_of;
    std::vector<std::vector<size_t>> groups;
    for (size_t j = 0; j < items.size(); j++) {
        const size_t g = group_of.emplace(refs[j], groups.size()).first->second;
        if (g == groups.size()) groups.emplace_back();
        groups[g].push_back(items[j]);
    }
    const size_t n = items.size();
    const size_t n_chunks = in.forced_chunks ? std::min<size_t>(in.forced_chunks, std::max<size_t>(1, n))
                                             : std::min<size_t>(ce_plan_ring_slots, std::max<size_t>(1, n / 64));
    size_t target = std::min((n + n_chunks - 1) / n_chunks, std::max<size_t>(1, in.budget / std::max<size_t>(in.per_pair, 1)));
    if (in.pooled_pairs < target && (size_t)in.pooled_pairs * 4 >= target * 3) target = in.pooled_pairs;
    std::vector<std::vector<size_t>> split;
    for (auto &g : groups)
        for (size_t o = 0; o < g.size(); o += target) split.emplace_back(g.begin() + o, g.begin() + std::min(g.size(), o + target));
    const bool several = n > target;
    size_t limit = (several && in.ramp && ring == 0) ? std::min(in.ramp, target) : target;
    const size_t bucket_begin = plan.size();
    for (size_t g0 = 0, g1 = 0; g0 < split.size(); g0 = g1) {
        size_t count = 0;
        while (g1 < split.size() && (count == 0 || count + split[g1].size() <= limit)) count += split[g1++].size();
        limit = std::min(target, limit * 2);
        ce_plan_chunk c{ring++ % ce_plan_ring_slots, (uint32_t)(several ? std::max(count, target) : count), ce_plan_none,
                        std::vector<std::vector<size_t>>(split.begin() + g0, split.begin() + g1)};
        for (size_t p = bucket_begin; p < plan.size(); p++)
            if (plan[p].slot == c.slot) c.collect_first = p;
        plan.push_back(std::move(c));
    }
}

struct ce_plan_entry {
    uint32_t tile, pair;
};

struct ce_xcd_keys {
    uint32_t channels;
    uint32_t keys_per_channel;
    uint32_t tiles_per_key;
    uint32_t round_to = 1;
};

inline bool operator==(const ce_xcd_keys &a, const ce_xcd_keys &b)
{
    return a.channels == b.channels && a.keys_per_channel == b.keys_per_channel && a.tiles_per_key == b.tiles_per_key &&
           a.round_to == b.round_to;
}

inline std::vector<ce_plan_entry> ce_plan_xcd_list(const uint32_t *pair_ref, uint32_t n_pairs, uint32_t n_refs, const ce_xcd_keys &k)
{
    std::vector<std::vector<uint32_t>> pairs_of(n_refs);
    for (uint32_t p = 0; p < n_pairs; p++) pairs_of[pair_ref[p]].push_back(p);
    std::vector<ce_plan_entry> cls[8];
    uint32_t key = 0;
    for (const auto &pairs : pairs_of) {
        if (pairs.empty()) continue;
        for (uint32_t c = 0; c < k.channels; c++)
            for (uint32_t j = 0; j < k.keys_per_channel; j++, key++)
                for (uint32_t sub = 0; sub < k.tiles_per_key; sub++)
                    for (uint32_t p : pairs) cls[key & 7].push_back({(j * k.tiles_per_key + sub) | c << 16, p});
    }
    size_t len = 0;
    for (const auto &v : cls) len = std::max(len, v.size());
    len = (len + k.round_to - 1) / k.round_to * k.round_to;
    std::vector<ce_plan_entry> list(len * 8, ce_plan_entry{~0u, 0u});
    for (uint32_t x = 0; x < 8; x++)
        for (size_t i = 0; i < cls[x].size(); i++) list[i * 8 + x] = cls[x][i];
    return list;
}

inline uint32_t ce_plan_dssim_levels(uint32_t w, uint32_t h, uint32_t max_levels, uint32_t *level_w, uint32_t *level_h)
{
    if (w == 0 || h == 0) return 0;
    uint32_t n = 0;
    while (n < max_levels) {
        level_w[n] = w;
        level_h[n] = h;
        n++;
        if (w < 8 || h < 8) break;
        w /= 2;
        h /= 2;
    }
    return n;
}

inline uint32_t ce_plan_ssim2_scales(uint32_t w, uint32_t h, uint32_t max_scales, uint32_t *scale_w, uint32_t *scale_h)
{
    uint32_t n = 0;
    for (uint32_t s = 0; s < max_scales; s++) {
        if (w < 8 || h < 8) break;
        if (s > 0) {
            w = w / 2 + (w & 1);
            h = h / 2 + (h & 1);
        }
        scale_w[n] = w;
        scale_h[n] = h;
        n++;
    }
    return n;
}
```

### codec-eval_amd/csrc/ce_ref_state.h

```cpp
#pragma once

#include <cstdint>
#include <cstring>

enum { CE_REF_SSIM2 = 0, CE_REF_DSSIM = 1, CE_REF_BUTTERAUGLI = 2, CE_REF_ROUNDTRIP = 3, CE_REF_KINDS = 4 };

inline uint64_t ce_ref_param_f32(float v)
{
    uint32_t u;
    std::memcpy(&u, &v, sizeof(u));
    return u;
}

struct ce_ref_state {
    const void *src = nullptr;
    uint32_t count = 0;
    uint64_t param = 0;
    bool covers(const void *slab, uint32_t n_refs, uint64_t p) const { return src && src == slab && n_refs <= count && param == p; }
    void invalidate() { src = nullptr, count = 0, param = 0; }
    void mark(const void *slab, uint32_t n_refs, uint64_t p) { src = slab, count = n_refs, param = p; }
};

struct ce_ref_states {
    bool keep = true;
    ce_ref_state of[CE_REF_KINDS];
    uint32_t builds[3] = {0, 0, 0};

    bool reuse(int k, const void *slab, uint32_t n_refs, uint64_t p)
    {
        if (keep && of[k].covers(slab, n_refs, p)) return true;
        of[k].invalidate();
        if (k < 3) builds[k]++;
        return false;
    }
    void built(int k, const void *slab, uint32_t n_refs, uint64_t p) { of[k].mark(slab, n_refs, p); }
    void invalidate()
    {
        for (auto &s : of) s.invalidate();
    }
};
```

### codec-eval_amd/csrc/ssim2.hip

```cpp
#include <algorithm>
#include <cstdlib>

#include "ce_internal.h"

namespace {

struct rg_consts {
    float mul_in[3];
    float mul_prev[3];
};

constexpr int kColsPerBlock = 64;

constexpr int kTailLevels = CE_MAX_SCALES - 1;
struct lvl_table {
    uint32_t n, first_level;
    uint32_t blk_end[kTailLevels];
    uint32_t w[kTailLevels], h[kTailLevels], pitch[kTailLevels];
    size_t plane[kTailLevels];
    const float *xyb[kTailLevels];
    float *hbuf[kTailLevels];
};

__device__ __forceinline__ uint32_t slot_of(uint32_t z, uint32_t n_refs_used, uint32_t max_refs)
{
    return z < n_refs_used ? z : max_refs + (z - n_refs_used);
}

__device__ __noinline__ float cbrt_f32_exact(float x)
{
    uint32_t hx = __float_as_uint(x) & 0x7fffffffu;
    if (hx == 0) return x;
    float t;
    if (hx < 0x00800000u) {
        t = __uint_as_float(0x4b800000u) * x;
        t = __uint_as_float((__float_as_uint(t) & 0x7fffffffu) / 3 + 642849266u);
    } else {
        t = __uint_as_float(hx / 3 + 709958130u);
    }
    double T = (double)t, r;
    const double xd = (double)x;
    r = T * T * T;
    T = T * (xd + xd + r) / (xd + r + r);
    r = T * T * T;
    T = T * (xd + xd + r) / (xd + r + r);
    return (float)T;
}

__device__ __forceinline__ float cbrt_f32(float x, uint32_t *slow = nullptr)
{
    if (x >= 1.0e-30f && x <= 1.0e30f) {
        const float s = __builtin_amdgcn_exp2f(__builtin_amdgcn_logf(x) * 0.333333343f);
        const double S = (double)s, xd = (double)x;
        const double s3 = S * S * S;
        const double diff = s3 - xd;
        const double inv0 = (double)__builtin_amdgcn_rcpf((float)s3);
        const double e = __builtin_fma(-s3, inv0, 1.0);
        const double inv = __builtin_fma(inv0, e, inv0);
        const double d = diff * inv;
        const double poly = __builtin_fma(d, 1.0 / 9.0, 1.0 / 3.0) * d;
        const double T = __builtin_fma(-S, poly, S);
        const int32_t low = (int32_t)((uint32_t)__double2loint(T) & 0x1fffffffu) - 0x10000000;
        if ((low < 0 ? -low : low) >= 0x4000) return (float)T;
    }
    if (slow) *slow += 1;
    return cbrt_f32_exact(x);
}

#define K_M00 0.30f
#define K_M02 0.078f
#define K_M01 (1.0f - K_M02 - K_M00)
#define K_M10 0.23f
#define K_M12 0.078f
#define K_M11 (1.0f - K_M12 - K_M10)
#define K_M20 0.24342268924547819f
#define K_M21 0.20476744424496821f
#define K_M22 (1.0f - K_M20 - K_M21)
#define K_B0 0.0037930732552754493f

__device__ __forceinline__ void linear_to_xyb_positive(float r, float g, float b, float cbrt_bias, float &X, float &Y,
                                                       float &B)
{
    const float m01 = K_M01, m11 = K_M11, m22 = K_M22;
    float m0 = __builtin_fmaf(K_M00, r, __builtin_fmaf(m01, g, __builtin_fmaf(K_M02, b, K_B0)));
    float m1 = __builtin_fmaf(K_M10, r, __builtin_fmaf(m11, g, __builtin_fmaf(K_M12, b, K_B0)));
    float m2 = __builtin_fmaf(K_M20, r, __builtin_fmaf(K_M21, g, __builtin_fmaf(m22, b, K_B0)));
    m0 = cbrt_f32(m0 < 0.0f ? 0.0f : m0) - cbrt_bias;
    m1 = cbrt_f32(m1 < 0.0f ? 0.0f : m1) - cbrt_bias;
    m2 = cbrt_f32(m2 < 0.0f ? 0.0f : m2) - cbrt_bias;
    X = 0.5f * (m0 - m1);
    Y = 0.5f * (m0 + m1);
    B = m2;
    B = (B - Y) + 0.55f;
    X = __builtin_fmaf(X, 14.0f, 0.42f);
    Y = Y + 0.01f;
}

template <int SRC>
__global__ __launch_bounds__(256) void k_ssim2_prep(const uint8_t *__restrict__ refs, const uint8_t *__restrict__ tests,
                                                    const float *__restrict__ lut, const float *__restrict__ lut_test,
                                                    const float *__restrict__ lin_in,
                                                    float *__restrict__ xyb, float *__restrict__ lin_out, uint32_t w,
                                                    uint32_t h, uint32_t pitch, size_t plane, uint32_t opitch,
                                                    size_t oplane, int has_next, size_t img_bytes, uint32_t n_refs_used,
                                                    uint32_t max_refs, uint32_t z0)
{
    constexpr bool FROM_U8 = SRC == CE_SRC_U8, FROM_U16 = SRC == CE_SRC_U16, FROM_LIN = SRC == CE_SRC_LIN;
    __shared__ float s_lut[256];
    if (FROM_U8) {
        s_lut[threadIdx.x] = lut[threadIdx.x];
        __syncthreads();
    }
    const uint32_t z = blockIdx.z + z0, slot = slot_of(z, n_refs_used, max_refs);
    const uint32_t qx = blockIdx.x * 64 + (threadIdx.x & 63), qy = blockIdx.y * 4 + (threadIdx.x >> 6);
    if (qx >= (w + 1) / 2 || qy >= (h + 1) / 2) return;
    const uint8_t *src8 = nullptr;
    if (FROM_U8 || FROM_U16 || FROM_LIN) src8 = z < n_refs_used ? refs + (size_t)z * img_bytes : tests + (size_t)(z - n_refs_used) * img_bytes;
    const uint16_t *src16 = reinterpret_cast<const uint16_t *>(src8);
    const float *tab16 = z < n_refs_used ? lut : lut_test;
    const float *srcf = lin_in + (size_t)slot * 3 * plane;
    const float cbrt_bias = cbrt_f32(K_B0);
    float sum[3] = {0.0f, 0.0f, 0.0f};
    float *xo = xyb + (size_t)slot * 3 * plane;
#pragma unroll
    for (uint32_t dy = 0; dy < 2; dy++) {
        const uint32_t yr = 2 * qy + dy, y = min(yr, h - 1);
        float X[2], Y[2], B[2];
        uint32_t lo = 0, hi = 0;
        if (FROM_U8) {
            const uintptr_t a = reinterpret_cast<uintptr_t>(src8 + ((size_t)y * w + 2 * qx) * 3);
            const uint32_t *q = reinterpret_cast<const uint32_t *>(a & ~(uintptr_t)3);
            const uint32_t d0 = q[0], d1 = q[1], d2 = q[2], sh = (uint32_t)(a & 3);
            lo = __builtin_amdgcn_alignbyte(d1, d0, sh);
            hi = __builtin_amdgcn_alignbyte(d2, d1, sh);
            if (2 * qx + 1 >= w) {
                hi = (lo >> 8) & 0xffffu;
                lo = (lo & 0x00ffffffu) | (lo << 24);
            }
        }
#pragma unroll
        for (uint32_t dx = 0; dx < 2; dx++) {
            const uint32_t xr = 2 * qx + dx, x = min(xr, w - 1);
            float r, g, bl;
            if (FROM_U8) {
                r = s_lut[dx ? lo >> 24 : lo & 255u];
                g = s_lut[dx ? hi & 255u : (lo >> 8) & 255u];
                bl = s_lut[dx ? (hi >> 8) & 255u : (lo >> 16) & 255u];
            } else if (FROM_U16) {
                const uint16_t *px = src16 + ((size_t)y * w + x) * 3;
                r = tab16[px[0]];
                g = tab16[px[1]];
                bl = tab16[px[2]];
            } else if (FROM_LIN) {
                const float *px = reinterpret_cast<const float *>(src8) + ((size_t)y * w + x) * 3;
                r = px[0];
                g = px[1];
                bl = px[2];
            } else {
                const size_t o = (size_t)y * pitch + x;
                r = srcf[o];
                g = srcf[o + plane];
                bl = srcf[o + 2 * plane];
            }
            sum[0] += r;
            sum[1] += g;
            sum[2] += bl;
            linear_to_xyb_positive(r, g, bl, cbrt_bias, X[dx], Y[dx], B[dx]);
        }
        if (yr < h) {
            const size_t o = (size_t)y * pitch + 2 * qx;
            if (2 * qx + 1 < w) {
                *reinterpret_cast<float2 *>(xo + o) = make_float2(X[0], X[1]);
                *reinterpret_cast<float2 *>(xo + o + plane) = make_float2(Y[0], Y[1]);
                *reinterpret_cast<float2 *>(xo + o + 2 * plane) = make_float2(B[0], B[1]);
            } else {
                xo[o] = X[0];
                xo[o + plane] = Y[0];
                xo[o + 2 * plane] = B[0];
            }
        }
    }
    if (has_next) {
        float *lo = lin_out + (size_t)slot * 3 * oplane + (size_t)qy * opitch + qx;
        lo[0] = sum[0] * 0.25f;
        lo[oplane] = sum[1] * 0.25f;
        lo[2 * oplane] = sum[2] * 0.25f;
    }
}

__device__ __forceinline__ float rg_step(float sum, float (&prev)[3], float (&prev2)[3], const rg_consts &rg)
{
    float o[3];
#pragma unroll
    for (int k = 0; k < 3; k++) {
        float v = sum * rg.mul_in[k];
        v = __builtin_fmaf(-1.0f, prev2[k], v);
        prev2[k] = prev[k];
        v = __builtin_fmaf(rg.mul_prev[k], prev[k], v);
        prev[k] = v;
        o[k] = v;
    }
    return o[0] + o[1] + o[2];
}

__device__ __forceinline__ void lds_barrier()
{
    asm volatile("" ::: "memory");
    __builtin_amdgcn_s_waitcnt(0xC07F);
    __builtin_amdgcn_s_barrier();
    asm volatile("" ::: "memory");
}

#ifndef CE_HB_ROWS
#define CE_HB_ROWS 32
#endif
constexpr int HB_ROWS = CE_HB_ROWS, HB_CW = 32, HB_LD = HB_ROWS + 1, HB_THREADS = 256;
constexpr int HB_LOADS = 2 * HB_ROWS * 8;
constexpr int HB_LSLOTS = (HB_LOADS + 63) / 64;
static_assert(HB_ROWS * CE_SSIM2_STREAMS <= HB_THREADS, "one task per thread");
constexpr int HB_HALF = HB_CW * HB_LD;
constexpr int HB_STORES = CE_SSIM2_STREAMS * HB_ROWS * (HB_CW / 4);

typedef float hb_f2 __attribute__((ext_vector_type(2)));

struct hblur_state {
    hb_f2 p01, q01;
    float p2, q2;
    float d[10];
};

__device__ __forceinline__ void hblur_chunk(const float *__restrict__ p_cur, const float *__restrict__ q_cur, bool plain,
                                            float *__restrict__ so, hblur_state &st, const rg_consts &rg)
{
    const hb_f2 n01 = {rg.mul_in[0], rg.mul_in[1]}, d01 = {rg.mul_prev[0], rg.mul_prev[1]};
#pragma unroll
    for (int half = 0; half < 2; half++) {
        float in[HB_CW / 2];
#pragma unroll
        for (int i = 0; i < HB_CW / 2; i++) in[i] = p_cur[(half * (HB_CW / 2) + i) * HB_LD];
#pragma unroll
        for (int i = 0; i < HB_CW / 2; i++) {
            const float q = q_cur[(half * (HB_CW / 2) + i) * HB_LD];
            in[i] = in[i] * (plain ? 1.0f : q);
        }
#pragma unroll
        for (int i = 0; i < HB_CW / 2; i++) {
            const int e = half * (HB_CW / 2) + i;
            const float sum = st.d[e % 10] + in[i];
            st.d[e % 10] = in[i];
            hb_f2 v01 = hb_f2{sum, sum} * n01;
            v01 = v01 - st.q01;
            st.q01 = st.p01;
            v01 = __builtin_elementwise_fma(d01, st.p01, v01);
            st.p01 = v01;
            float v2 = sum * rg.mul_in[2];
            v2 = v2 - st.q2;
            st.q2 = st.p2;
            v2 = __builtin_fmaf(rg.mul_prev[2], st.p2, v2);
            st.p2 = v2;
            so[e * HB_LD] = v01.x + v01.y + v2;
        }
    }
    float t[10];
#pragma unroll
    for (int j = 0; j < 10; j++) t[j] = st.d[(j + HB_CW) % 10];
#pragma unroll
    for (int j = 0; j < 10; j++) st.d[j] = t[j];
}

template <int LEVEL>
__global__ __launch_bounds__(HB_THREADS) void k_ssim2_hblur_lds(const float *__restrict__ xyb,
                                                                const uint32_t *__restrict__ pair_ref,
                                                                float *__restrict__ hbuf, uint32_t w, uint32_t h,
                                                                uint32_t pitch, size_t plane, uint32_t max_refs,
                                                                rg_consts rg, lvl_table tab, const uint2 *__restrict__ work,
                                                                const uint32_t *__restrict__ pair_first)
{
    __shared__ float s_in[2][2 * HB_HALF];
    __shared__ float s_out[CE_SSIM2_STREAMS * HB_HALF];
    const uint32_t tid = threadIdx.x, lane = tid & 63, wv = tid >> 6;
    uint32_t bx = blockIdx.x, c = blockIdx.y, p = blockIdx.z;
    if (work) {
        const uint2 wi = work[blockIdx.x];
        if (wi.x == ~0u) return;
        bx = wi.x & 0xffffu, c = wi.x >> 16, p = wi.y;
    }
    if (LEVEL < 0) {
        uint32_t l = 0;
        while (l + 1 < tab.n && bx >= tab.blk_end[l]) l++;
        bx -= l ? tab.blk_end[l - 1] : 0;
        xyb = tab.xyb[l], hbuf = tab.hbuf[l];
        w = tab.w[l], h = tab.h[l], pitch = tab.pitch[l], plane = tab.plane[l];
    }
    const uint32_t y0 = bx * HB_ROWS;
    const float *ga = xyb + ((size_t)pair_ref[p] * 3 + c) * plane;
    const float *gb = xyb + ((size_t)(max_refs + p) * 3 + c) * plane;
    const int n_chunks = (int)(pitch / HB_CW);
    const bool loader = wv == 3;
    const float *l_src[HB_LSLOTS];
    uint32_t l_dst[HB_LSLOTS];
    uint32_t l_row[HB_LSLOTS];
    const uint32_t lq = lane & 7;
#pragma unroll
    for (int m = 0; m < HB_LSLOTS; m++) {
        const uint32_t j = min(64u * m + lane, (uint32_t)HB_LOADS - 1), pl = j / (HB_ROWS * 8), row = (j % (HB_ROWS * 8)) >> 3;
        l_row[m] = 64u * m + lane < (uint32_t)HB_LOADS ? y0 + row : ~0u;
        l_src[m] = (pl ? gb : ga) + (size_t)min(y0 + row, h - 1) * pitch;
        l_dst[m] = pl * (2 * HB_HALF) + (4 * lq) * HB_LD + row;
    }
    float4 pf[HB_LSLOTS];
    auto load_chunk = [&](int k) {
        if (loader) {
            const int col = max(HB_CW * k - 28 + 4 * (int)lq, 0);
#pragma unroll
            for (int m = 0; m < HB_LSLOTS; m++) pf[m] = *reinterpret_cast<const float4 *>(l_src[m] + col);
        }
    };
    auto stash_chunk = [&](int k) {
        if (loader) {
            const int col = HB_CW * k - 28 + 4 * (int)lq;
            float *base = &s_in[0][0] + (k & 1) * HB_HALF;
#pragma unroll
            for (int m = 0; m < HB_LSLOTS; m++) {
                if (l_row[m] == ~0u) continue;
                float *dst = base + l_dst[m];
                const bool rv = l_row[m] < h && col >= 0;
                dst[0] = (rv && col < (int)w) ? pf[m].x : 0.0f;
                dst[HB_LD] = (rv && col + 1 < (int)w) ? pf[m].y : 0.0f;
                dst[2 * HB_LD] = (rv && col + 2 < (int)w) ? pf[m].z : 0.0f;
                dst[3 * HB_LD] = (rv && col + 3 < (int)w) ? pf[m].w : 0.0f;
            }
        }
    };

    load_chunk(0);
    stash_chunk(0);
    if (n_chunks > 1) load_chunk(1);
    __syncthreads();

    const bool full = pair_first[p] == p;
    const uint32_t n_jobs = full ? CE_SSIM2_STREAMS : 3;
    const bool worker = tid < n_jobs * HB_ROWS;
    const uint32_t tj = worker ? tid / HB_ROWS : 0, tr = worker ? tid % HB_ROWS : 0;
    const uint32_t ts = full ? tj : (tj == 0 ? 1u : tj + 2u);
    const bool plain = ts < 2;
    const float *sp = &s_in[(ts == 1 || ts == 3) ? 1 : 0][tr];
    const float *sq = &s_in[(ts == 2) ? 0 : 1][tr];
    float *so = &s_out[ts * HB_HALF + tr];
    hblur_state st;
    st.p01 = st.q01 = hb_f2{0.0f, 0.0f};
    st.p2 = st.q2 = 0.0f;
#pragma unroll
    for (int j = 0; j < 10; j++) st.d[j] = 0.0f;
    float *obase = hbuf + ((size_t)p * 3 + c) * CE_SSIM2_STREAMS * plane;

    for (int k = 0; k < n_chunks; k++) {
        if (k + 1 < n_chunks) stash_chunk(k + 1);
        if (k + 2 < n_chunks) load_chunk(k + 2);
        const uint32_t oc = (k & 1) * HB_HALF;
        if (worker) hblur_chunk(sp + oc, sq + oc, plain, so, st, rg);
        lds_barrier();
        if (k > 0 && !loader) {
#pragma unroll
            for (int it = 0; it < (HB_STORES + 191) / 192; it++) {
                const uint32_t idx = it * 192 + tid;
                if (idx >= n_jobs * (HB_ROWS * 8)) break;
                const uint32_t oj = idx / (HB_ROWS * 8), rem = idx % (HB_ROWS * 8), orow = rem >> 3, oq = rem & 7;
                const uint32_t os = full ? oj : (oj == 0 ? 1u : oj + 2u);
                const float *src = &s_out[os * HB_HALF + (4 * oq) * HB_LD + orow];
                const float4 v = make_float4(src[0], src[HB_LD], src[2 * HB_LD], src[3 * HB_LD]);
                if (y0 + orow < h)
                    *reinterpret_cast<float4 *>(obase + (size_t)os * plane + (size_t)(y0 + orow) * pitch + HB_CW * (k - 1) + 4 * oq) = v;
            }
        }
        lds_barrier();
    }
}

__device__ __forceinline__ double wave_sum(double v)
{
#pragma unroll
    for (int off = 32; off > 0; off >>= 1) v += __shfl_down(v, off, 64);
    return v;
}

constexpr int VB_G = 4;
constexpr int VB_PLANES = 7;
constexpr int VB_SLOT = VB_G * 64;
constexpr int VB_GROUP = VB_PLANES * VB_SLOT;

struct vblur_state {
    float prev[CE_SSIM2_STREAMS][3], prev2[CE_SSIM2_STREAMS][3];
    float rr[16][CE_SSIM2_STREAMS];
    double acc[6];
};

template <int GG, bool CHECKED, bool STORE>
__device__ __forceinline__ void vblur_group(vblur_state &st, const float *__restrict__ slot, int g, uint32_t h,
                                            const rg_consts &rg, float *__restrict__ map, uint32_t pitch, size_t plane,
                                            uint32_t lane, bool active)
{
    const float C2 = 0.0009f;
    float gacc[6] = {0.f, 0.f, 0.f, 0.f, 0.f, 0.f};
#pragma unroll
    for (int e = 0; e < VB_G; e++) {
        const uint32_t i = (uint32_t)(4 * g + e);
        constexpr int base = 4 * GG;
        const int re = base + e;
        float v[CE_SSIM2_STREAMS];
#pragma unroll
        for (int s = 0; s < CE_SSIM2_STREAMS; s++) {
            const float ld = slot[s * VB_SLOT + e * 64];
            const float right = (!CHECKED || i < h) ? ld : 0.0f;
            const float left = st.rr[(re + 6) & 15][s];
            st.rr[re][s] = right;
            v[s] = rg_step(left + right, st.prev[s], st.prev2[s], rg);
        }
        if (!CHECKED || (i >= 4 && i < h + 4)) {
            const float img1 = slot[5 * VB_SLOT + e * 64], img2 = slot[6 * VB_SLOT + e * 64];
            const float mu1 = v[0], mu2 = v[1], s11 = v[2], s22 = v[3], s12 = v[4];
            const float mu11 = mu1 * mu1, mu22 = mu2 * mu2, mu12 = mu1 * mu2;
            const float mu_diff = mu1 - mu2;
            const float num_m = __builtin_fmaf(mu_diff, -mu_diff, 1.0f);
            const float num_s = __builtin_fmaf(2.0f, s12 - mu12, C2);
            const float denom_s = (s11 - mu11) + (s22 - mu22) + C2;
            float d = 1.0f - (num_m * num_s) / denom_s;
            d = d > 0.0f ? d : 0.0f;
            const float dd = d * d;
            const float e1 = fabsf(img1 - mu1), e2 = fabsf(img2 - mu2);
            const float d1 = (e2 - e1) * __builtin_amdgcn_rcpf(1.0f + e1);
            const float artifact = d1 > 0.0f ? d1 : 0.0f;
            const float detail = d1 < 0.0f ? -d1 : 0.0f;
            const float aa = artifact * artifact, ll = detail * detail;
            if (STORE && active) {
                float *row = map + (size_t)(i - 4) * pitch;
                row[lane] = d;
                (row + plane)[lane] = artifact;
                (row + 2 * plane)[lane] = detail;
            }
            gacc[0] += d;
            gacc[1] += dd * dd;
            gacc[2] += artifact;
            gacc[3] += aa * aa;
            gacc[4] += detail;
            gacc[5] += ll * ll;
        }
    }
#pragma unroll
    for (int q = 0; q < 6; q++) st.acc[q] += (double)gacc[q];
}

struct ssim2_map_table {
    float *lvl[CE_MAX_SCALES];
};

template <int LEVEL, bool STORE>
__global__ __launch_bounds__(64) void k_ssim2_vblur_dma(const float *__restrict__ hbuf, const float *__restrict__ xyb,
                                                        const uint32_t *__restrict__ pair_ref,
                                                        double *__restrict__ partials, uint32_t w, uint32_t h,
                                                        uint32_t pitch, size_t plane, uint32_t max_refs, uint32_t scale,
                                                        uint32_t max_vblocks, rg_consts rg, lvl_table tab,
                                                        const uint2 *__restrict__ work, const uint32_t *__restrict__ pair_first,
                                                        ssim2_map_table maps)
{
    __shared__ __attribute__((aligned(16))) float ring[2 * VB_GROUP];
    uint32_t bx = blockIdx.x, c = blockIdx.y, p = blockIdx.z;
    if (work) {
        const uint2 wi = work[blockIdx.x];
        if (wi.x == ~0u) return;
        bx = wi.x & 0xffffu, c = wi.x >> 16, p = wi.y;
    }
    if (LEVEL < 0) {
        uint32_t l = 0;
        while (l + 1 < tab.n && bx >= tab.blk_end[l]) l++;
        bx -= l ? tab.blk_end[l - 1] : 0;
        xyb = tab.xyb[l], hbuf = tab.hbuf[l];
        w = tab.w[l], h = tab.h[l], pitch = tab.pitch[l], plane = tab.plane[l];
        scale = tab.first_level + l;
    }
    const uint32_t lane = threadIdx.x, x0 = bx * 64;
    const bool active = x0 + lane < w;
    const float *hb = hbuf + ((size_t)p * 3 + c) * CE_SSIM2_STREAMS * plane + x0;
    const float *hb_ref = hbuf + ((size_t)pair_first[p] * 3 + c) * CE_SSIM2_STREAMS * plane + x0;
    const float *xa = xyb + ((size_t)pair_ref[p] * 3 + c) * plane + x0;
    const float *xb = xyb + ((size_t)(max_refs + p) * 3 + c) * plane + x0;
    const uint32_t dr = lane >> 4, dc = (lane & 15) * 4;
    float *map = STORE ? maps.lvl[scale] + ((size_t)p * 9 + (size_t)c * 3) * plane + x0 : nullptr;

    using gptr = const __attribute__((address_space(1))) void *;
    using lptr = __attribute__((address_space(3))) void *;
    auto issue_group = [&](int g) {
        float *dst = ring + (g & 1) * VB_GROUP;
        const uint32_t row = min((uint32_t)(4 * g) + dr, h - 1);
        const size_t off = (size_t)row * pitch + dc;
#pragma unroll
        for (int s = 0; s < CE_SSIM2_STREAMS; s++)
            __builtin_amdgcn_global_load_lds((gptr)(((s == 0 || s == 2) ? hb_ref : hb) + (size_t)s * plane + off), (lptr)(dst + s * VB_SLOT), 16, 0, 0);
        const int rx = 4 * g - 4 + (int)dr;
        const size_t offx = (size_t)min((uint32_t)max(rx, 0), h - 1) * pitch + dc;
        __builtin_amdgcn_global_load_lds((gptr)(xa + offx), (lptr)(dst + 5 * VB_SLOT), 16, 0, 0);
        __builtin_amdgcn_global_load_lds((gptr)(xb + offx), (lptr)(dst + 6 * VB_SLOT), 16, 0, 0);
    };

    vblur_state st;
#pragma unroll
    for (int s = 0; s < CE_SSIM2_STREAMS; s++) {
#pragma unroll
        for (int k = 0; k < 3; k++) st.prev[s][k] = st.prev2[s][k] = 0.0f;
#pragma unroll
        for (int e = 0; e < 16; e++) st.rr[e][s] = 0.0f;
    }
#pragma unroll
    for (int q = 0; q < 6; q++) st.acc[q] = 0.0;
    const int n_groups = (int)((h + 4 + VB_G - 1) / VB_G);
    const int full_groups = (int)(h / VB_G);

    issue_group(0);
    issue_group(1);
#define CE_VGROUP(GG, CHECKED)                                                                         \
    do {                                                                                               \
                    \
        asm volatile("s_waitcnt vmcnt(7)" ::: "memory");                                               \
        vblur_group<GG, CHECKED, STORE>(st, ring + ((GG) & 1) * VB_GROUP + lane, g0 + (GG), h, rg, map, \
                                        pitch, plane, lane, active);                                   \
                      \
        asm volatile("s_waitcnt lgkmcnt(0)" ::: "memory");                                             \
        issue_group(g0 + (GG) + 2);                                                                    \
    } while (0)
    int g0 = 0;
    {
        CE_VGROUP(0, true);
        CE_VGROUP(1, true);
        if (2 < n_groups) CE_VGROUP(2, true);
        if (3 < n_groups) CE_VGROUP(3, true);
        g0 = 4;
    }
    for (; g0 + 3 < full_groups; g0 += 4) {
        CE_VGROUP(0, false);
        CE_VGROUP(1, false);
        CE_VGROUP(2, false);
        CE_VGROUP(3, false);
    }
    for (; g0 < n_groups; g0 += 4) {
        CE_VGROUP(0, true);
        if (g0 + 1 < n_groups) CE_VGROUP(1, true);
        if (g0 + 2 < n_groups) CE_VGROUP(2, true);
        if (g0 + 3 < n_groups) CE_VGROUP(3, true);
    }
#undef CE_VGROUP
    asm volatile("s_waitcnt vmcnt(0)" ::: "memory");
    double *dst = partials + ((((size_t)p * CE_MAX_SCALES + scale) * 3 + c) * max_vblocks + bx) * 6;
#pragma unroll
    for (int q = 0; q < 6; q++) {
        const double sum = wave_sum(active ? st.acc[q] : 0.0);
        if (lane == 0) dst[q] = sum;
    }
}

__global__ __launch_bounds__(256) void k_cbrt_sweep(uint32_t first, uint64_t count, unsigned long long *out)
{
    uint64_t mism = 0, slow = 0;
    for (uint64_t i = (uint64_t)blockIdx.x * blockDim.x + threadIdx.x; i < count; i += (uint64_t)gridDim.x * blockDim.x) {
        const float x = __uint_as_float(first + (uint32_t)i);
        uint32_t sl = 0;
        const float a = cbrt_f32(x, &sl), b = cbrt_f32_exact(x);
        mism += __float_as_uint(a) != __float_as_uint(b);
        slow += sl;
    }
    if (mism) atomicAdd(out, (unsigned long long)mism);
    if (slow) atomicAdd(out + 1, (unsigned long long)slow);
}

__constant__ double c_weight[108] = {
    0.0, 0.0007376606707406586, 0.0, 0.0, 0.0007793481682867309, 0.0, 0.0, 0.0004371155730107379, 0.0, 1.1041726426657346, 0.00066284834129271, 0.00015231632783718752,
    0.0, 0.0016406437456599754, 0.0, 1.8422455520539298, 11.441172603757666, 0.0, 0.0007989109436015163, 0.000176816438078653, 0.0, 1.8787594979546387, 10.94906990605142, 0.0,
    0.0007289346991508072, 0.9677937080626833, 0.0, 0.00014003424285435884, 0.9981766977854967, 0.00031949755934435053, 0.0004550992113792063, 0.0, 0.0, 0.0013648766163243398, 0.0, 0.0,
    0.0, 0.0, 0.0, 7.466890328078848, 0.0, 17.445833984131262, 0.0006235601634041466, 0.0, 0.0, 6.683678146179332, 0.00037724407979611296, 1.027889937768264,
    225.20515300849274, 0.0, 0.0, 19.213238186143016, 0.0011401524586618361, 0.001237755635509985, 176.39317598450694, 0.0, 0.0, 24.43300999870476, 0.28520802612117757, 0.0004485436923833408,
    0.0, 0.0, 0.0, 34.77906344483772, 44.835625328877896, 0.0, 0.0, 0.0, 0.0, 0.0, 0.0, 0.0,
    0.0, 0.0008680556573291698, 0.0, 0.0, 0.0, 0.0, 0.0, 0.0005313191874358747, 0.0, 0.00016533814161379112, 0.0, 0.0,
    0.0, 0.0, 0.0, 0.0004179171803251336, 0.0017290828234722833, 0.0, 0.0020827005846636437, 0.0, 0.0, 8.826982764996862, 23.19243343998926, 0.0,
    95.1080498811086, 0.9863978034400682, 0.9834382792465353, 0.0012286405048278493, 171.2667255897307, 0.9807858872435379, 0.0, 0.0, 0.0, 0.0005130064588990679, 0.0, 0.00010854057858411537,
};

struct scale_geom {
    uint32_t npix[CE_MAX_SCALES];
    uint32_t nblk[CE_MAX_SCALES];
};

__global__ __launch_bounds__(128) void k_ssim2_finalize(const double *__restrict__ partials, double *__restrict__ avg,
                                                        ce_dev_scores *__restrict__ scores, uint32_t n_scales,
                                                        uint32_t max_vblocks, scale_geom g)
{
    __shared__ double s_avg[CE_MAX_SCALES * 3 * 6];
    const uint32_t p = blockIdx.x, t = threadIdx.x;
    if (t < n_scales * 18) {
        const uint32_t s = t / 18, c = (t / 6) % 3, q = t % 6;
        const double *src = partials + ((((size_t)p * CE_MAX_SCALES + s) * 3 + c) * max_vblocks) * 6 + q;
        double sum = 0.0;
        for (uint32_t k = 0; k < g.nblk[s]; k++) sum += src[(size_t)k * 6];
        const double one_per_pixels = 1.0 / (double)g.npix[s];
        double v = one_per_pixels * sum;
        if (q & 1) v = sqrt(sqrt(v));
        s_avg[t] = v;
        avg[(size_t)p * CE_MAX_SCALES * 18 + t] = v;
    }
    __syncthreads();
    if (t == 0) {
        double ssim = 0.0;
        int i = 0;
        for (uint32_t c = 0; c < 3; c++)
            for (uint32_t s = 0; s < n_scales; s++) {
                const double *a = s_avg + (s * 3 + c) * 6;
                for (int n = 0; n < 2; n++) {
                    ssim = fma(c_weight[i++], fabs(a[0 + n]), ssim);
                    ssim = fma(c_weight[i++], fabs(a[2 + n]), ssim);
                    ssim = fma(c_weight[i++], fabs(a[4 + n]), ssim);
                }
            }
        ssim *= 0.9562382616834844;
        ssim = fma(6.248496625763138e-5 * ssim * ssim, ssim,
                   fma(2.326765642916932, ssim, -0.020884521182843837 * ssim * ssim));
        if (ssim > 0.0)
            ssim = fma(pow(ssim, 0.6276336467831387), -10.0, 100.0);
        else
            ssim = 100.0;
        scores[p].ssimulacra2 = ssim;
    }
}

}


void ce_ssim2_free(ce_batch *b)
{
    for (int s = 0; s < CE_MAX_SCALES; s++) {
        hipFree(b->d_lin[s]);
        hipFree(b->d_xyb[s]);
        hipFree(b->d_hbuf[s]);
        b->d_lin[s] = b->d_xyb[s] = b->d_hbuf[s] = nullptr;
        if (b->lvl_stream[s]) hipStreamSynchronize(b->lvl_stream[s]);
        if (b->ev_prep[s]) hipEventDestroy(b->ev_prep[s]);
        if (b->ev_done[s]) hipEventDestroy(b->ev_done[s]);
        b->lvl_stream[s] = nullptr;
        b->ev_prep[s] = b->ev_done[s] = nullptr;
    }
    hipFree(b->d_partials);
    hipFree(b->d_avg);
    hipFree(b->s2_map);
    hipFree(b->s2_cells);
    b->d_partials = nullptr;
    b->d_avg = nullptr;
    b->s2_map = b->s2_cells = nullptr;
    for (int s = 0; s < CE_MAX_SCALES; s++) b->s2_map_lvl[s] = nullptr;
    b->s2_cells_cap = 0;
    b->s2_map_pairs = b->s2_norm_pairs = 0;
    for (ce_xcd_list *L : {&b->work_h, &b->work_v, &b->work_ht, &b->work_vt}) ce_free_xcd_list(L);
    b->refs.of[CE_REF_SSIM2].invalidate();
    b->ssim2_ready = false;
}

static int ssim2_allocate(ce_batch *b)
{
    ce_ctx *ctx = b->ctx;
    const int ns = b->n_scales;
    const size_t slots = (size_t)b->max_refs + b->max_pairs;
    for (int s = 1; s < ns; s++)
        CE_HIP(ctx, hipMalloc(&b->d_lin[s], slots * 3 * b->sd[s].plane * sizeof(float)));
    for (int s = 0; s < ns; s++) {
        CE_HIP(ctx, hipMalloc(&b->d_xyb[s], slots * 3 * b->sd[s].plane * sizeof(float)));
        CE_HIP(ctx, hipMalloc(&b->d_hbuf[s], (size_t)b->max_pairs * 3 * CE_SSIM2_STREAMS * b->sd[s].plane * sizeof(float)));
        if (s == 0 && !(b->lvl_stream[0] = ce_ctx_aux_stream(ctx, ce_ctx::AUX_SSIM2_L0))) return CE_ERR_BACKEND;
        CE_HIP(ctx, hipEventCreateWithFlags(&b->ev_prep[s], hipEventDisableTiming));
        CE_HIP(ctx, hipEventCreateWithFlags(&b->ev_done[s], hipEventDisableTiming));
    }
    b->max_vblocks = (b->sd[0].w + kColsPerBlock - 1) / kColsPerBlock;
    CE_HIP(ctx, hipMalloc(&b->d_partials, (size_t)b->max_pairs * CE_MAX_SCALES * 3 * b->max_vblocks * 6 * sizeof(double)));
    CE_HIP(ctx, hipMalloc(&b->d_avg, (size_t)b->max_pairs * CE_MAX_SCALES * 18 * sizeof(double)));
    return CE_OK;
}

int ce_ssim2_prepare(ce_batch *b)
{
    if (b->ssim2_ready) return CE_OK;
    uint32_t sw[CE_MAX_SCALES], sh[CE_MAX_SCALES];
    const int ns = (int)ce_plan_ssim2_scales(b->w, b->h, CE_MAX_SCALES, sw, sh);
    for (int s = 0; s < ns; s++) {
        const uint32_t w = sw[s], h = sh[s];
        ce_scale_dims &d = b->sd[s];
        d.w = w;
        d.h = h;
        d.pitch = ((w + HB_CW - 1) / HB_CW) * HB_CW + HB_CW;
        d.plane = (size_t)d.pitch * (((size_t)h + HB_ROWS - 1) / HB_ROWS * HB_ROWS);
        d.hpitch = d.pitch;
        d.hplane = d.plane;
    }
    b->n_scales = ns;
    if (ns == 0) return CE_OK;
    const int rc = ssim2_allocate(b);
    if (rc != CE_OK) {
        const std::string why = b->ctx->err;
        ce_ssim2_free(b);
        (void)hipGetLastError();
        b->ctx->err = why;
        return rc;
    }
    b->ssim2_ready = true;
    return CE_OK;
}

static int build_pass_list(ce_batch *b, uint32_t n_pairs, uint32_t n_blocks, ce_xcd_list *L)
{
    if (n_blocks > 0xffffu) {
        b->ctx->err = "SSIMULACRA2: image too large for the block index of the work list";
        return CE_ERR_INVALID_ARG;
    }
    return ce_build_xcd_list(b, n_pairs, ce_xcd_keys{3, n_blocks, 1}, L);
}

int ce_launch_ssim2(ce_batch *b, const uint8_t *d_refs, uint32_t n_refs_used, uint32_t n_pairs, bool store_maps)
{
    ce_ctx *ctx = b->ctx;
    int rc = ce_ssim2_prepare(b);
    if (rc != CE_OK) return rc;
    ssim2_map_table maps{};
    if (store_maps) {
        if (!b->s2_map) {
            size_t total = 0;
            for (int s = 0; s < b->n_scales; s++) total += (size_t)b->max_pairs * 9 * b->sd[s].plane;
            if (hipMalloc(&b->s2_map, total * sizeof(float)) != hipSuccess) {
                b->s2_map = nullptr;
                (void)hipGetLastError();
                ctx->err = "out of device memory for the SSIMULACRA2 maps";
                return CE_ERR_BACKEND;
            }
            size_t off = 0;
            for (int s = 0; s < b->n_scales; s++) {
                b->s2_map_lvl[s] = b->s2_map + off;
                off += (size_t)b->max_pairs * 9 * b->sd[s].plane;
            }
        }
        for (int s = 0; s < b->n_scales; s++) maps.lvl[s] = b->s2_map_lvl[s];
    }
    rg_consts rg;
    ce_ssim2_recursive_gaussian(rg.mul_in, rg.mul_prev);
    const uint32_t n_slots = n_refs_used + n_pairs;
    const int levels = std::min(b->n_scales, b->debug_max_scales);
    const bool cached = b->refs.reuse(CE_REF_SSIM2, d_refs, n_refs_used, (uint64_t)levels);
    const uint32_t z0 = cached ? n_refs_used : 0;
    using hblur_fn = void (*)(const float *, const uint32_t *, float *, uint32_t, uint32_t, uint32_t, size_t, uint32_t,
                              rg_consts, lvl_table, const uint2 *, const uint32_t *);
    using vblur_fn = void (*)(const float *, const float *, const uint32_t *, double *, uint32_t, uint32_t, uint32_t,
                              size_t, uint32_t, uint32_t, uint32_t, rg_consts, lvl_table, const uint2 *, const uint32_t *,
                              ssim2_map_table);
    const hblur_fn h_l0 = k_ssim2_hblur_lds<0>, h_tail = k_ssim2_hblur_lds<-1>;
    const vblur_fn v_l0 = k_ssim2_vblur_dma<0, false>, v_tail = k_ssim2_vblur_dma<-1, false>;
    const vblur_fn v_l0_map = k_ssim2_vblur_dma<0, true>, v_tail_map = k_ssim2_vblur_dma<-1, true>;
    scale_geom g{};
    hipStream_t s0 = ctx->prof_serial ? CE_STREAM(ctx) : b->lvl_stream[0];
    hipStream_t s1 = CE_STREAM(ctx);
    lvl_table tab{};
    lvl_table tab_v{};
    for (int s = 0; s < levels; s++) {
        const ce_scale_dims &d = b->sd[s];
        const bool has_next = s + 1 < levels;
        const ce_scale_dims &nd = b->sd[has_next ? s + 1 : s];
        const dim3 quad_grid(((d.w + 1) / 2 + 63) / 64, ((d.h + 1) / 2 + 3) / 4, n_slots - z0);
        if (s == 0 && b->linear)
            CE_LAUNCH(ctx, "ssim2_prep_lin", k_ssim2_prep<CE_SRC_LIN>, quad_grid, dim3(256), 0, d_refs, b->d_tests, (const float *)nullptr,
                      (const float *)nullptr, (const float *)nullptr, b->d_xyb[0], b->d_lin[1], d.w, d.h, d.pitch, d.plane, nd.pitch,
                      nd.plane, has_next ? 1 : 0, b->img_bytes, n_refs_used, b->max_refs, z0);
        else if (s == 0 && b->depth[0])
            CE_LAUNCH(ctx, "ssim2_prep_u16", k_ssim2_prep<CE_SRC_U16>, quad_grid, dim3(256), 0, d_refs, b->d_tests, b->deep_lut[0][0],
                      b->deep_lut[0][1], (const float *)nullptr, b->d_xyb[0], b->d_lin[1], d.w, d.h, d.pitch, d.plane, nd.pitch,
                      nd.plane, has_next ? 1 : 0, b->img_bytes, n_refs_used, b->max_refs, z0);
        else if (s == 0)
            CE_LAUNCH(ctx, "ssim2_prep_u8", k_ssim2_prep<CE_SRC_U8>, quad_grid, dim3(256), 0, d_refs, b->d_tests, ctx->d_lut_ssim2, ctx->d_lut_ssim2,
                      (const float *)nullptr, b->d_xyb[0], b->d_lin[1], d.w, d.h, d.pitch, d.plane, nd.pitch, nd.plane,
                      has_next ? 1 : 0, b->img_bytes, n_refs_used, b->max_refs, z0);
        else
            CE_LAUNCH(ctx, "ssim2_prep", k_ssim2_prep<CE_SRC_F32>, quad_grid, dim3(256), 0, d_refs, b->d_tests, ctx->d_lut_ssim2, ctx->d_lut_ssim2,
                      (const float *)b->d_lin[s], b->d_xyb[s], b->d_lin[has_next ? s + 1 : s], d.w, d.h, d.pitch, d.plane,
                      nd.pitch, nd.plane, has_next ? 1 : 0, b->img_bytes, n_refs_used, b->max_refs, z0);
        const uint32_t hblk = (d.h + HB_ROWS - 1) / HB_ROWS, vblk = (d.w + kColsPerBlock - 1) / kColsPerBlock;
        g.npix[s] = d.w * d.h;
        g.nblk[s] = vblk;
        if (s == 0) {
            if (s0 != CE_STREAM(ctx)) {
                CE_HIP(ctx, hipEventRecord(b->ev_prep[0], CE_STREAM(ctx)));
                CE_HIP(ctx, hipStreamWaitEvent(s0, b->ev_prep[0], 0));
            }
            if ((rc = build_pass_list(b, n_pairs, hblk, &b->work_h)) != CE_OK) return rc;
            if ((rc = build_pass_list(b, n_pairs, vblk, &b->work_v)) != CE_OK) return rc;
            CE_LAUNCH_ON(ctx, s0, "ssim2_hblur_L0", h_l0, dim3(b->work_h.len), dim3(HB_THREADS), 0, b->d_xyb[0], b->d_pair_ref,
                         b->d_hbuf[0], d.w, d.h, d.pitch, d.plane, b->max_refs, rg, tab, (const uint2 *)b->work_h.d,
                         (const uint32_t *)b->d_pair_first);
#define CE_VBLUR_L0_ARGS                                                                                                   \
    b->d_hbuf[0], b->d_xyb[0], b->d_pair_ref, b->d_partials, d.w, d.h, d.pitch, d.plane, b->max_refs, 0u, b->max_vblocks, rg, tab, \
        (const uint2 *)b->work_v.d, (const uint32_t *)b->d_pair_first, maps
            if (store_maps)
                CE_LAUNCH_ON(ctx, s0, "ssim2_vblur_ssim_map_L0", v_l0_map, dim3(b->work_v.len), dim3(64), 0, CE_VBLUR_L0_ARGS);
            else
                CE_LAUNCH_ON(ctx, s0, "ssim2_vblur_ssim_L0", v_l0, dim3(b->work_v.len), dim3(64), 0, CE_VBLUR_L0_ARGS);
#undef CE_VBLUR_L0_ARGS
            if (s0 != CE_STREAM(ctx)) CE_HIP(ctx, hipEventRecord(b->ev_done[0], s0));
        } else {
            const uint32_t l = tab.n++;
            tab_v.n = tab.n;
            tab.first_level = tab_v.first_level = 1;
            tab.blk_end[l] = (l ? tab.blk_end[l - 1] : 0) + hblk;
            tab_v.blk_end[l] = (l ? tab_v.blk_end[l - 1] : 0) + vblk;
            tab.w[l] = tab_v.w[l] = d.w;
            tab.h[l] = tab_v.h[l] = d.h;
            tab.pitch[l] = tab_v.pitch[l] = d.pitch;
            tab.plane[l] = tab_v.plane[l] = d.plane;
            tab.xyb[l] = tab_v.xyb[l] = b->d_xyb[s];
            tab.hbuf[l] = tab_v.hbuf[l] = b->d_hbuf[s];
        }
    }
    if (tab.n) {
        if (s1 != CE_STREAM(ctx)) {
            CE_HIP(ctx, hipEventRecord(b->ev_prep[1], CE_STREAM(ctx)));
            CE_HIP(ctx, hipStreamWaitEvent(s1, b->ev_prep[1], 0));
        }
        if ((rc = build_pass_list(b, n_pairs, tab.blk_end[tab.n - 1], &b->work_ht)) != CE_OK) return rc;
        if ((rc = build_pass_list(b, n_pairs, tab_v.blk_end[tab_v.n - 1], &b->work_vt)) != CE_OK) return rc;
        CE_LAUNCH_ON(ctx, s1, "ssim2_hblur_L1-5", h_tail, dim3(b->work_ht.len), dim3(HB_THREADS), 0,
                     (const float *)nullptr, b->d_pair_ref, (float *)nullptr, 0u, 0u, 0u, (size_t)0, b->max_refs, rg, tab,
                     (const uint2 *)b->work_ht.d, (const uint32_t *)b->d_pair_first);
#define CE_VBLUR_TAIL_ARGS                                                                                                  \
    (const float *)nullptr, (const float *)nullptr, b->d_pair_ref, b->d_partials, 0u, 0u, 0u, (size_t)0, b->max_refs, 0u,        \
        b->max_vblocks, rg, tab_v, (const uint2 *)b->work_vt.d, (const uint32_t *)b->d_pair_first, maps
        if (store_maps)
            CE_LAUNCH_ON(ctx, s1, "ssim2_vblur_ssim_map_L1-5", v_tail_map, dim3(b->work_vt.len), dim3(64), 0, CE_VBLUR_TAIL_ARGS);
        else
            CE_LAUNCH_ON(ctx, s1, "ssim2_vblur_ssim_L1-5", v_tail, dim3(b->work_vt.len), dim3(64), 0, CE_VBLUR_TAIL_ARGS);
#undef CE_VBLUR_TAIL_ARGS
        if (s1 != CE_STREAM(ctx)) CE_HIP(ctx, hipEventRecord(b->ev_done[1], s1));
    }
    if (s0 != CE_STREAM(ctx)) {
        CE_HIP(ctx, hipStreamWaitEvent(CE_STREAM(ctx), b->ev_done[0], 0));
        if (tab.n && s1 != CE_STREAM(ctx)) CE_HIP(ctx, hipStreamWaitEvent(CE_STREAM(ctx), b->ev_done[1], 0));
    }
    CE_LAUNCH(ctx, "ssim2_finalize", k_ssim2_finalize, dim3(n_pairs), dim3(128), 0, b->d_partials, b->d_avg,
              b->d_scores, (uint32_t)levels, b->max_vblocks, g);
    CE_HIP(ctx, hipGetLastError());
    if (!cached) b->refs.built(CE_REF_SSIM2, d_refs, n_refs_used, (uint64_t)levels);
    return CE_OK;
}

int ce_ssim2_cbrt_sweep(ce_ctx *ctx, uint32_t first_bits, uint64_t count, uint64_t *mismatches, uint64_t *slow_path)
{
    unsigned long long *d = nullptr, h[2] = {0, 0};
    CE_HIP(ctx, hipMalloc(&d, sizeof(h)));
    CE_HIP(ctx, hipMemsetAsync(d, 0, sizeof(h), ctx->stream));
    CE_LAUNCH(ctx, "cbrt_sweep", k_cbrt_sweep, dim3(4096), dim3(256), 0, first_bits, count, d);
    CE_HIP(ctx, hipMemcpyAsync(h, d, sizeof(h), hipMemcpyDeviceToHost, ctx->stream));
    CE_HIP(ctx, hipStreamSynchronize(ctx->stream));
    CE_HIP(ctx, hipFree(d));
    if (mismatches) *mismatches = h[0];
    if (slow_path) *slow_path = h[1];
    return CE_OK;
}

int ce_ssim2_read_maps(ce_batch *b, uint32_t scale, uint32_t channel, uint32_t kind, uint32_t first, uint32_t count,
                       uint32_t block, float *maps, double *norms)
{
    ce_ctx *ctx = b->ctx;
    if (norms) {
        CE_HIP(ctx, hipMemcpy2DAsync(norms, 2 * sizeof(double), b->d_avg + (size_t)first * CE_MAX_SCALES * 18 + scale * 18 + channel * 6 + 2 * kind,
                                     CE_MAX_SCALES * 18 * sizeof(double), 2 * sizeof(double), count, hipMemcpyDeviceToHost, ctx->stream));
        if (!maps) CE_HIP(ctx, hipStreamSynchronize(ctx->stream));
    }
    if (!maps) return CE_OK;
    const ce_scale_dims &d = b->sd[scale];
    return ce_read_map_cells(b, "ssim2_block_max", b->s2_map_lvl[scale] + (size_t)(channel * 3 + kind) * d.plane,
                             ce_map_geom{d.w, d.h, d.pitch, 9 * d.plane}, first, count, block, false, &b->s2_cells, &b->s2_cells_cap,
                             maps);
}

int ce_ssim2_occupancy(int which)
{
    int n = -1;
    if (which == 0)
        hipOccupancyMaxActiveBlocksPerMultiprocessor(&n, k_ssim2_hblur_lds<0>, HB_THREADS, 0);
    else
        hipOccupancyMaxActiveBlocksPerMultiprocessor(&n, k_ssim2_vblur_dma<0, false>, 64, 0);
    return n;
}
```

Baseline: 21070.

## Cache fully blurred SSIMULACRA2 reference planes and skip per-pair reference blurs

Adds a split path for SSIMULACRA2. It precomputes the fully blurred reference mu and sigma planes once per reference into a new per-batch buffer, and the per-pair horizontal blur then computes only the three test-dependent streams. The vertical blur kernel reads the cached reference planes directly instead of blurring them per pair. The path is gated by reference reuse, ref handles and an env var. It costs extra device memory for the cached planes and extra build kernels the first time a reference is seen.

```diff
diff --git a/codec-eval_amd/csrc/ce_api.cpp b/codec-eval_amd/csrc/ce_api.cpp
--- a/codec-eval_amd/csrc/ce_api.cpp
+++ b/codec-eval_amd/csrc/ce_api.cpp
@@ -797,14 +797,14 @@
 }
 
 
-size_t ce_estimate_batch_bytes(uint32_t w, uint32_t h, uint32_t n_refs, uint32_t n_pairs, uint32_t metric_mask)
+static size_t estimate_batch_bytes(uint32_t w, uint32_t h, uint32_t n_refs, uint32_t n_pairs, uint32_t metric_mask, bool ref_planes)
 {
     const double px = (double)w * h, slots = (double)n_refs + n_pairs, pairs = n_pairs;
     double bytes = 3.0 * px * slots + 64.0 * pairs;
     double allocations = 8;
     if (metric_mask & CE_METRIC_SSIMULACRA2) {
-        bytes += px * (20.0 * slots + 80.0 * pairs);
-        allocations += 24;
+        bytes += px * (20.0 * slots + 80.0 * pairs + (ref_planes ? 32.0 * n_refs : 0.0));
+        allocations += ref_planes ? 30 : 24;
     }
     if (metric_mask & CE_METRIC_DSSIM) {
         bytes += px * (6.0 * slots + 48.0 * n_refs + 17.4 * pairs);
@@ -816,6 +816,11 @@
     }
     if (metric_mask & CE_METRIC_PSNR) bytes += 8.0 * pairs;
     return (size_t)(bytes * 1.2) + (size_t)(allocations * (256u << 10)) + (8u << 20);
+}
+
+size_t ce_estimate_batch_bytes(uint32_t w, uint32_t h, uint32_t n_refs, uint32_t n_pairs, uint32_t metric_mask)
+{
+    return estimate_batch_bytes(w, h, n_refs, n_pairs, metric_mask, true);
 }
 
 size_t ce_estimate_batch_bytes_deep(uint32_t w, uint32_t h, uint32_t n_refs, uint32_t n_pairs, uint32_t metric_mask, uint32_t ref_depth,
@@ -872,7 +877,7 @@
         const ce_batch *pb = kv.second;
         const uint32_t held = (pb->ssim2_ready ? CE_METRIC_SSIMULACRA2 : 0u) | (pb->dssim_ready ? CE_METRIC_DSSIM : 0u) |
                               (pb->ba_ready ? CE_METRIC_BUTTERAUGLI : 0u);
-        pooled += ce_estimate_batch_bytes(pb->w, pb->h, pb->max_refs, pb->max_pairs, held);
+        pooled += estimate_batch_bytes(pb->w, pb->h, pb->max_refs, pb->max_pairs, held, pb->s2_ref_blur[0] != nullptr);
     }
     const size_t share = (size_t)((double)(free_b + pooled) * 0.8 / ce_ctx::kPoolRing);
     return std::min(share, ce_ctx::kChunkBytesMax);
@@ -997,8 +1002,8 @@
         const uint32_t w = it->first.first, h = it->first.second;
         std::vector<const void *> refs;
         for (size_t i : it->second) refs.push_back(pairs[i].reference);
-        const size_t per_pair = ce_estimate_batch_bytes(w, h, 1, 2, metric_mask) - ce_estimate_batch_bytes(w, h, 1, 1, metric_mask) +
-                                ce_estimate_batch_bytes(w, h, 2, 1, metric_mask) - ce_estimate_batch_bytes(w, h, 1, 1, metric_mask);
+        const size_t per_pair = estimate_batch_bytes(w, h, 1, 2, metric_mask, false) - estimate_batch_bytes(w, h, 1, 1, metric_mask, false) +
+                                estimate_batch_bytes(w, h, 2, 1, metric_mask, false) - estimate_batch_bytes(w, h, 1, 1, metric_mask, false);
         auto pooled = ctx->shape_pool.find(std::make_tuple(w, h, 0u));
         const ce_plan_inputs in{chunk_budget(ctx), per_pair, pooled != ctx->shape_pool.end() ? pooled->second->max_pairs : 0u, forced_chunks, ramp0};
         const size_t first = plan.size();
@@ -1176,6 +1181,7 @@
         return rc;
     }
     b->refs.keep = true;
+    b->ref_handle = true;
     *out = new ce_ref{ctx, b, flags};
     return CE_OK;
 }
@@ -1198,6 +1204,7 @@
         CE_HIP(ctx, hipStreamSynchronize(ctx->stream));
         ce_invalidate_reference_state(nb);
         nb->refs.keep = true;
+        nb->ref_handle = true;
         for (int k = 0; k < 3; k++) nb->refs.builds[k] = b->refs.builds[k];
         ce_batch_destroy(b);
         ref->batch = b = nb;
@@ -1384,6 +1391,7 @@
         case 4:
             if (channel < 0 || channel > 2) return CE_ERR_INVALID_ARG;
             src = b->d_hbuf[scale] + (size_t)channel * CE_SSIM2_STREAMS * d.hplane;
+            if (b->s2_split_last) return ce_fail(ctx, CE_ERR_INVALID_ARG, "the last launch took SSIMULACRA2's split path: it leaves no row-blurred reference streams to read");
             break;
         default: return CE_ERR_INVALID_ARG;
     }
diff --git a/codec-eval_amd/csrc/ce_internal.h b/codec-eval_amd/csrc/ce_internal.h
--- a/codec-eval_amd/csrc/ce_internal.h
+++ b/codec-eval_amd/csrc/ce_internal.h
@@ -146,6 +146,8 @@
     float *d_lin[CE_MAX_SCALES] = {};
     float *d_xyb[CE_MAX_SCALES] = {};
     float *d_hbuf[CE_MAX_SCALES] = {};
+    float *s2_ref_blur[CE_MAX_SCALES] = {};
+    bool s2_split_last = false, ref_handle = false;
     hipStream_t lvl_stream[CE_MAX_SCALES] = {};
     hipStream_t metric_stream[3] = {};
     hipEvent_t ev_fork = nullptr, ev_join[3] = {};
diff --git a/codec-eval_amd/csrc/ce_plan.h b/codec-eval_amd/csrc/ce_plan.h
--- a/codec-eval_amd/csrc/ce_plan.h
+++ b/codec-eval_amd/csrc/ce_plan.h
@@ -95,6 +95,17 @@
     return list;
 }
 
+enum { CE_SSIM2_BLUR_TODAY = 0, CE_SSIM2_BLUR_SPLIT = 1, CE_SSIM2_BLUR_SPLIT_BUILD = 2 };
+
+inline int ce_plan_ssim2_ref_blur(bool enabled, bool keeps_state, bool handle, bool reused, bool covered, uint32_t n_pairs,
+                                  uint32_t n_refs)
+{
+    if (!enabled || !keeps_state) return CE_SSIM2_BLUR_TODAY;
+    if (covered) return CE_SSIM2_BLUR_SPLIT;
+    if (handle) return CE_SSIM2_BLUR_SPLIT_BUILD;
+    return (reused && n_pairs > n_refs) ? CE_SSIM2_BLUR_SPLIT_BUILD : CE_SSIM2_BLUR_TODAY;
+}
+
 inline uint32_t ce_plan_dssim_levels(uint32_t w, uint32_t h, uint32_t max_levels, uint32_t *level_w, uint32_t *level_h)
 {
     if (w == 0 || h == 0) return 0;
diff --git a/codec-eval_amd/csrc/ce_ref_state.h b/codec-eval_amd/csrc/ce_ref_state.h
--- a/codec-eval_amd/csrc/ce_ref_state.h
+++ b/codec-eval_amd/csrc/ce_ref_state.h
@@ -3,7 +3,7 @@
 #include <cstdint>
 #include <cstring>
 
-enum { CE_REF_SSIM2 = 0, CE_REF_DSSIM = 1, CE_REF_BUTTERAUGLI = 2, CE_REF_ROUNDTRIP = 3, CE_REF_KINDS = 4 };
+enum { CE_REF_SSIM2 = 0, CE_REF_DSSIM = 1, CE_REF_BUTTERAUGLI = 2, CE_REF_ROUNDTRIP = 3, CE_REF_SSIM2_BLUR = 4, CE_REF_KINDS = 5 };
 
 inline uint64_t ce_ref_param_f32(float v)
 {
diff --git a/codec-eval_amd/csrc/ssim2.hip b/codec-eval_amd/csrc/ssim2.hip
--- a/codec-eval_amd/csrc/ssim2.hip
+++ b/codec-eval_amd/csrc/ssim2.hip
@@ -268,7 +268,9 @@
     for (int j = 0; j < 10; j++) st.d[j] = t[j];
 }
 
-template <int LEVEL>
+enum { HB_BY_FIRST = 0, HB_PAIR3 = 1, HB_REF2 = 2 };
+
+template <int LEVEL, int JOBS = HB_BY_FIRST>
 __global__ __launch_bounds__(HB_THREADS) void k_ssim2_hblur_lds(const float *__restrict__ xyb,
                                                                 const uint32_t *__restrict__ pair_ref,
                                                                 float *__restrict__ hbuf, uint32_t w, uint32_t h,
@@ -293,8 +295,8 @@
         w = tab.w[l], h = tab.h[l], pitch = tab.pitch[l], plane = tab.plane[l];
     }
     const uint32_t y0 = bx * HB_ROWS;
-    const float *ga = xyb + ((size_t)pair_ref[p] * 3 + c) * plane;
-    const float *gb = xyb + ((size_t)(max_refs + p) * 3 + c) * plane;
+    const float *ga = xyb + ((size_t)(JOBS == HB_REF2 ? p : pair_ref[p]) * 3 + c) * plane;
+    const float *gb = JOBS == HB_REF2 ? ga : xyb + ((size_t)(max_refs + p) * 3 + c) * plane;
     const int n_chunks = (int)(pitch / HB_CW);
     const bool loader = wv == 3;
     const float *l_src[HB_LSLOTS];
@@ -338,11 +340,11 @@
     if (n_chunks > 1) load_chunk(1);
     __syncthreads();
 
-    const bool full = pair_first[p] == p;
-    const uint32_t n_jobs = full ? CE_SSIM2_STREAMS : 3;
+    const bool full = JOBS == HB_BY_FIRST && pair_first[p] == p;
+    const uint32_t n_jobs = JOBS == HB_REF2 ? 2 : full ? CE_SSIM2_STREAMS : 3;
     const bool worker = tid < n_jobs * HB_ROWS;
     const uint32_t tj = worker ? tid / HB_ROWS : 0, tr = worker ? tid % HB_ROWS : 0;
-    const uint32_t ts = full ? tj : (tj == 0 ? 1u : tj + 2u);
+    const uint32_t ts = JOBS == HB_REF2 ? 2u * tj : full ? tj : (tj == 0 ? 1u : tj + 2u);
     const bool plain = ts < 2;
     const float *sp = &s_in[(ts == 1 || ts == 3) ? 1 : 0][tr];
     const float *sq = &s_in[(ts == 2) ? 0 : 1][tr];
@@ -352,7 +354,7 @@
     st.p2 = st.q2 = 0.0f;
 #pragma unroll
     for (int j = 0; j < 10; j++) st.d[j] = 0.0f;
-    float *obase = hbuf + ((size_t)p * 3 + c) * CE_SSIM2_STREAMS * plane;
+    float *obase = hbuf + ((size_t)p * 3 + c) * (JOBS == HB_REF2 ? 2 : CE_SSIM2_STREAMS) * plane;
 
     for (int k = 0; k < n_chunks; k++) {
         if (k + 1 < n_chunks) stash_chunk(k + 1);
@@ -366,11 +368,12 @@
                 const uint32_t idx = it * 192 + tid;
                 if (idx >= n_jobs * (HB_ROWS * 8)) break;
                 const uint32_t oj = idx / (HB_ROWS * 8), rem = idx % (HB_ROWS * 8), orow = rem >> 3, oq = rem & 7;
-                const uint32_t os = full ? oj : (oj == 0 ? 1u : oj + 2u);
+                const uint32_t os = JOBS == HB_REF2 ? 2u * oj : full ? oj : (oj == 0 ? 1u : oj + 2u);
+                const uint32_t op = JOBS == HB_REF2 ? oj : os;
                 const float *src = &s_out[os * HB_HALF + (4 * oq) * HB_LD + orow];
                 const float4 v = make_float4(src[0], src[HB_LD], src[2 * HB_LD], src[3 * HB_LD]);
                 if (y0 + orow < h)
-                    *reinterpret_cast<float4 *>(obase + (size_t)os * plane + (size_t)(y0 + orow) * pitch + HB_CW * (k - 1) + 4 * oq) = v;
+                    *reinterpret_cast<float4 *>(obase + (size_t)op * plane + (size_t)(y0 + orow) * pitch + HB_CW * (k - 1) + 4 * oq) = v;
             }
         }
         lds_barrier();
@@ -395,7 +398,7 @@
     double acc[6];
 };
 
-template <int GG, bool CHECKED, bool STORE>
+template <int GG, bool CHECKED, bool STORE, bool REFB>
 __device__ __forceinline__ void vblur_group(vblur_state &st, const float *__restrict__ slot, int g, uint32_t h,
                                             const rg_consts &rg, float *__restrict__ map, uint32_t pitch, size_t plane,
                                             uint32_t lane, bool active)
@@ -410,6 +413,7 @@
         float v[CE_SSIM2_STREAMS];
 #pragma unroll
         for (int s = 0; s < CE_SSIM2_STREAMS; s++) {
+            if (REFB && (s == 0 || s == 2)) continue;
             const float ld = slot[s * VB_SLOT + e * 64];
             const float right = (!CHECKED || i < h) ? ld : 0.0f;
             const float left = st.rr[(re + 6) & 15][s];
@@ -418,7 +422,8 @@
         }
         if (!CHECKED || (i >= 4 && i < h + 4)) {
             const float img1 = slot[5 * VB_SLOT + e * 64], img2 = slot[6 * VB_SLOT + e * 64];
-            const float mu1 = v[0], mu2 = v[1], s11 = v[2], s22 = v[3], s12 = v[4];
+            const float mu1 = REFB ? slot[0 * VB_SLOT + e * 64] : v[0], s11 = REFB ? slot[2 * VB_SLOT + e * 64] : v[2];
+            const float mu2 = v[1], s22 = v[3], s12 = v[4];
             const float mu11 = mu1 * mu1, mu22 = mu2 * mu2, mu12 = mu1 * mu2;
             const float mu_diff = mu1 - mu2;
             const float num_m = __builtin_fmaf(mu_diff, -mu_diff, 1.0f);
@@ -454,14 +459,18 @@
     float *lvl[CE_MAX_SCALES];
 };
 
-template <int LEVEL, bool STORE>
+struct ssim2_ref_table {
+    float *lvl[CE_MAX_SCALES];
+};
+
+template <int LEVEL, bool STORE, bool REFB = false>
 __global__ __launch_bounds__(64) void k_ssim2_vblur_dma(const float *__restrict__ hbuf, const float *__restrict__ xyb,
                                                         const uint32_t *__restrict__ pair_ref,
                                                         double *__restrict__ partials, uint32_t w, uint32_t h,
                                                         uint32_t pitch, size_t plane, uint32_t max_refs, uint32_t scale,
                                                         uint32_t max_vblocks, rg_consts rg, lvl_table tab,
                                                         const uint2 *__restrict__ work, const uint32_t *__restrict__ pair_first,
-                                                        ssim2_map_table maps)
+                                                        ssim2_map_table maps, ssim2_ref_table refb)
 {
     __shared__ __attribute__((aligned(16))) float ring[2 * VB_GROUP];
     uint32_t bx = blockIdx.x, c = blockIdx.y, p = blockIdx.z;
@@ -481,7 +490,8 @@
     const uint32_t lane = threadIdx.x, x0 = bx * 64;
     const bool active = x0 + lane < w;
     const float *hb = hbuf + ((size_t)p * 3 + c) * CE_SSIM2_STREAMS * plane + x0;
-    const float *hb_ref = hbuf + ((size_t)pair_first[p] * 3 + c) * CE_SSIM2_STREAMS * plane + x0;
+    const float *hb_ref = REFB ? nullptr : hbuf + ((size_t)pair_first[p] * 3 + c) * CE_SSIM2_STREAMS * plane + x0;
+    const float *fin = REFB ? refb.lvl[scale] + ((size_t)pair_ref[p] * 3 + c) * 2 * plane + x0 : nullptr;
     const float *xa = xyb + ((size_t)pair_ref[p] * 3 + c) * plane + x0;
     const float *xb = xyb + ((size_t)(max_refs + p) * 3 + c) * plane + x0;
     const uint32_t dr = lane >> 4, dc = (lane & 15) * 4;
@@ -493,6 +503,18 @@
         float *dst = ring + (g & 1) * VB_GROUP;
         const uint32_t row = min((uint32_t)(4 * g) + dr, h - 1);
         const size_t off = (size_t)row * pitch + dc;
+        if (REFB) {
+            const int rx = 4 * g - 4 + (int)dr;
+            const size_t offx = (size_t)min((uint32_t)max(rx, 0), h - 1) * pitch + dc;
+#pragma unroll
+            for (int s = 0; s < CE_SSIM2_STREAMS; s++) {
+                const float *from = (s == 0 || s == 2) ? fin + (size_t)(s >> 1) * plane + offx : hb + (size_t)s * plane + off;
+                __builtin_amdgcn_global_load_lds((gptr)from, (lptr)(dst + s * VB_SLOT), 16, 0, 0);
+            }
+            __builtin_amdgcn_global_load_lds((gptr)(xa + offx), (lptr)(dst + 5 * VB_SLOT), 16, 0, 0);
+            __builtin_amdgcn_global_load_lds((gptr)(xb + offx), (lptr)(dst + 6 * VB_SLOT), 16, 0, 0);
+            return;
+        }
 #pragma unroll
         for (int s = 0; s < CE_SSIM2_STREAMS; s++)
             __builtin_amdgcn_global_load_lds((gptr)(((s == 0 || s == 2) ? hb_ref : hb) + (size_t)s * plane + off), (lptr)(dst + s * VB_SLOT), 16, 0, 0);
@@ -521,7 +543,7 @@
     do {                                                                                               \
                     \
         asm volatile("s_waitcnt vmcnt(7)" ::: "memory");                                               \
-        vblur_group<GG, CHECKED, STORE>(st, ring + ((GG) & 1) * VB_GROUP + lane, g0 + (GG), h, rg, map, \
+        vblur_group<GG, CHECKED, STORE, REFB>(st, ring + ((GG) & 1) * VB_GROUP + lane, g0 + (GG), h, rg, map, \
                                         pitch, plane, lane, active);                                   \
                       \
         asm volatile("s_waitcnt lgkmcnt(0)" ::: "memory");                                             \
@@ -557,6 +579,57 @@
     }
 }
 
+template <int LEVEL>
+__global__ __launch_bounds__(64) void k_ssim2_ref_vblur(const float *__restrict__ hin, float *__restrict__ out, uint32_t w, uint32_t h,
+                                                        uint32_t pitch, size_t plane, rg_consts rg, lvl_table tab,
+                                                        ssim2_ref_table hins, ssim2_ref_table outs)
+{
+    uint32_t bx = blockIdx.x;
+    const uint32_t c = blockIdx.y, r = blockIdx.z;
+    if (LEVEL < 0) {
+        uint32_t l = 0;
+        while (l + 1 < tab.n && bx >= tab.blk_end[l]) l++;
+        bx -= l ? tab.blk_end[l - 1] : 0;
+        hin = hins.lvl[tab.first_level + l], out = outs.lvl[tab.first_level + l];
+        w = tab.w[l], h = tab.h[l], pitch = tab.pitch[l], plane = tab.plane[l];
+    }
+    const uint32_t x = bx * 64 + threadIdx.x;
+    if (x >= w) return;
+    const float *src = hin + ((size_t)r * 3 + c) * 2 * plane + x;
+    float *dst = out + ((size_t)r * 3 + c) * 2 * plane + x;
+    float prev[2][3], prev2[2][3], rr[16][2];
+#pragma unroll
+    for (int s = 0; s < 2; s++) {
+#pragma unroll
+        for (int k = 0; k < 3; k++) prev[s][k] = prev2[s][k] = 0.0f;
+#pragma unroll
+        for (int e = 0; e < 16; e++) rr[e][s] = 0.0f;
+    }
+    for (uint32_t i0 = 0; i0 < h + 4; i0 += 16) {
+        float in[16][2];
+#pragma unroll
+        for (int e = 0; e < 16; e++) {
+            const size_t row = (size_t)min(i0 + e, h - 1) * pitch;
+            in[e][0] = src[row], in[e][1] = src[plane + row];
+        }
+#pragma unroll
+        for (int e = 0; e < 16; e++) {
+            const uint32_t i = i0 + e;
+            if (i < h + 4) {
+#pragma unroll
+                for (int s = 0; s < 2; s++) {
+                    const float right = i < h ? in[e][s] : 0.0f;
+                    const float left = rr[(e + 6) & 15][s];
+                    rr[e][s] = right;
+                    const float v = rg_step(left + right, prev[s], prev2[s], rg);
+                    if (i >= 4) dst[(size_t)s * plane] = v;
+                }
+                if (i >= 4) dst += pitch;
+            }
+        }
+    }
+}
+
 __global__ __launch_bounds__(256) void k_cbrt_sweep(uint32_t first, uint64_t count, unsigned long long *out)
 {
     uint64_t mism = 0, slow = 0;
@@ -638,7 +711,8 @@
         hipFree(b->d_lin[s]);
         hipFree(b->d_xyb[s]);
         hipFree(b->d_hbuf[s]);
-        b->d_lin[s] = b->d_xyb[s] = b->d_hbuf[s] = nullptr;
+        hipFree(b->s2_ref_blur[s]);
+        b->d_lin[s] = b->d_xyb[s] = b->d_hbuf[s] = b->s2_ref_blur[s] = nullptr;
         if (b->lvl_stream[s]) hipStreamSynchronize(b->lvl_stream[s]);
         if (b->ev_prep[s]) hipEventDestroy(b->ev_prep[s]);
         if (b->ev_done[s]) hipEventDestroy(b->ev_done[s]);
@@ -657,6 +731,8 @@
     b->s2_map_pairs = b->s2_norm_pairs = 0;
     for (ce_xcd_list *L : {&b->work_h, &b->work_v, &b->work_ht, &b->work_vt}) ce_free_xcd_list(L);
     b->refs.of[CE_REF_SSIM2].invalidate();
+    b->refs.of[CE_REF_SSIM2_BLUR].invalidate();
+    b->s2_split_last = false;
     b->ssim2_ready = false;
 }
 
@@ -678,6 +754,21 @@
     CE_HIP(ctx, hipMalloc(&b->d_partials, (size_t)b->max_pairs * CE_MAX_SCALES * 3 * b->max_vblocks * 6 * sizeof(double)));
     CE_HIP(ctx, hipMalloc(&b->d_avg, (size_t)b->max_pairs * CE_MAX_SCALES * 18 * sizeof(double)));
     return CE_OK;
+}
+
+static bool ssim2_ref_blur_allocate(ce_batch *b)
+{
+    if (b->s2_ref_blur[0]) return true;
+    for (int s = 0; s < b->n_scales; s++)
+        if (hipMalloc(&b->s2_ref_blur[s], (size_t)b->max_refs * 3 * 2 * b->sd[s].plane * sizeof(float)) != hipSuccess) {
+            (void)hipGetLastError();
+            for (int t = 0; t < b->n_scales; t++) {
+                hipFree(b->s2_ref_blur[t]);
+                b->s2_ref_blur[t] = nullptr;
+            }
+            return false;
+        }
+    return true;
 }
 
 int ce_ssim2_prepare(ce_batch *b)
@@ -748,12 +839,27 @@
     const int levels = std::min(b->n_scales, b->debug_max_scales);
     const bool cached = b->refs.reuse(CE_REF_SSIM2, d_refs, n_refs_used, (uint64_t)levels);
     const uint32_t z0 = cached ? n_refs_used : 0;
+    static const bool ref_blur_enabled = [] { const char *e = std::getenv("CE_SSIM2_REF_BLUR"); return !(e && e[0] == '0'); }();
+    if (!cached) b->refs.of[CE_REF_SSIM2_BLUR].invalidate();
+    const bool blur_covered = b->refs.keep && b->refs.of[CE_REF_SSIM2_BLUR].covers(d_refs, n_refs_used, (uint64_t)levels);
+    int blur_path = ce_plan_ssim2_ref_blur(ref_blur_enabled, b->refs.keep, b->ref_handle, cached, blur_covered, n_pairs, n_refs_used);
+    if (blur_path == CE_SSIM2_BLUR_SPLIT_BUILD && (size_t)n_refs_used * 2 > (size_t)b->max_pairs * CE_SSIM2_STREAMS) blur_path = CE_SSIM2_BLUR_TODAY;
+    if (blur_path == CE_SSIM2_BLUR_SPLIT_BUILD && !ssim2_ref_blur_allocate(b)) blur_path = CE_SSIM2_BLUR_TODAY;
+    const bool split = blur_path != CE_SSIM2_BLUR_TODAY, build_ref = blur_path == CE_SSIM2_BLUR_SPLIT_BUILD;
+    if (build_ref) b->refs.of[CE_REF_SSIM2_BLUR].invalidate();
+    b->s2_split_last = split;
+    ssim2_ref_table ref_h{}, ref_blur{};
+    for (int s = 0; s < b->n_scales; s++) ref_h.lvl[s] = b->d_hbuf[s], ref_blur.lvl[s] = b->s2_ref_blur[s];
     using hblur_fn = void (*)(const float *, const uint32_t *, float *, uint32_t, uint32_t, uint32_t, size_t, uint32_t,
                               rg_consts, lvl_table, const uint2 *, const uint32_t *);
     using vblur_fn = void (*)(const float *, const float *, const uint32_t *, double *, uint32_t, uint32_t, uint32_t,
                               size_t, uint32_t, uint32_t, uint32_t, rg_consts, lvl_table, const uint2 *, const uint32_t *,
-                              ssim2_map_table);
-    const hblur_fn h_l0 = k_ssim2_hblur_lds<0>, h_tail = k_ssim2_hblur_lds<-1>;
+                              ssim2_map_table, ssim2_ref_table);
+    const hblur_fn h_l0 = split ? k_ssim2_hblur_lds<0, HB_PAIR3> : k_ssim2_hblur_lds<0>;
+    const hblur_fn h_tail = split ? k_ssim2_hblur_lds<-1, HB_PAIR3> : k_ssim2_hblur_lds<-1>;
+    const hblur_fn h_l0_ref = k_ssim2_hblur_lds<0, HB_REF2>, h_tail_ref = k_ssim2_hblur_lds<-1, HB_REF2>;
+    const vblur_fn vr_l0 = k_ssim2_vblur_dma<0, false, true>, vr_tail = k_ssim2_vblur_dma<-1, false, true>;
+    const vblur_fn vr_l0_map = k_ssim2_vblur_dma<0, true, true>, vr_tail_map = k_ssim2_vblur_dma<-1, true, true>;
     const vblur_fn v_l0 = k_ssim2_vblur_dma<0, false>, v_tail = k_ssim2_vblur_dma<-1, false>;
     const vblur_fn v_l0_map = k_ssim2_vblur_dma<0, true>, v_tail_map = k_ssim2_vblur_dma<-1, true>;
     scale_geom g{};
@@ -792,13 +898,24 @@
             }
             if ((rc = build_pass_list(b, n_pairs, hblk, &b->work_h)) != CE_OK) return rc;
             if ((rc = build_pass_list(b, n_pairs, vblk, &b->work_v)) != CE_OK) return rc;
+            if (build_ref) {
+                CE_LAUNCH_ON(ctx, s0, "ssim2_ref_hblur_L0", h_l0_ref, dim3(hblk, 3, n_refs_used), dim3(HB_THREADS), 0, b->d_xyb[0], b->d_pair_ref,
+                             b->d_hbuf[0], d.w, d.h, d.pitch, d.plane, b->max_refs, rg, tab, (const uint2 *)nullptr,
+                             (const uint32_t *)b->d_pair_first);
+                CE_LAUNCH_ON(ctx, s0, "ssim2_ref_vblur_L0", k_ssim2_ref_vblur<0>, dim3(vblk, 3, n_refs_used), dim3(64), 0,
+                             (const float *)b->d_hbuf[0], b->s2_ref_blur[0], d.w, d.h, d.pitch, d.plane, rg, tab, ref_h, ref_blur);
+            }
             CE_LAUNCH_ON(ctx, s0, "ssim2_hblur_L0", h_l0, dim3(b->work_h.len), dim3(HB_THREADS), 0, b->d_xyb[0], b->d_pair_ref,
                          b->d_hbuf[0], d.w, d.h, d.pitch, d.plane, b->max_refs, rg, tab, (const uint2 *)b->work_h.d,
                          (const uint32_t *)b->d_pair_first);
 #define CE_VBLUR_L0_ARGS                                                                                                   \
     b->d_hbuf[0], b->d_xyb[0], b->d_pair_ref, b->d_partials, d.w, d.h, d.pitch, d.plane, b->max_refs, 0u, b->max_vblocks, rg, tab, \
-        (const uint2 *)b->work_v.d, (const uint32_t *)b->d_pair_first, maps
-            if (store_maps)
+        (const uint2 *)b->work_v.d, (const uint32_t *)b->d_pair_first, maps, ref_blur
+            if (split && store_maps)
+                CE_LAUNCH_ON(ctx, s0, "ssim2_vblur_ssim_map_L0", vr_l0_map, dim3(b->work_v.len), dim3(64), 0, CE_VBLUR_L0_ARGS);
+            else if (split)
+                CE_LAUNCH_ON(ctx, s0, "ssim2_vblur_ssim_L0", vr_l0, dim3(b->work_v.len), dim3(64), 0, CE_VBLUR_L0_ARGS);
+            else if (store_maps)
                 CE_LAUNCH_ON(ctx, s0, "ssim2_vblur_ssim_map_L0", v_l0_map, dim3(b->work_v.len), dim3(64), 0, CE_VBLUR_L0_ARGS);
             else
                 CE_LAUNCH_ON(ctx, s0, "ssim2_vblur_ssim_L0", v_l0, dim3(b->work_v.len), dim3(64), 0, CE_VBLUR_L0_ARGS);
@@ -825,13 +942,24 @@
         }
         if ((rc = build_pass_list(b, n_pairs, tab.blk_end[tab.n - 1], &b->work_ht)) != CE_OK) return rc;
         if ((rc = build_pass_list(b, n_pairs, tab_v.blk_end[tab_v.n - 1], &b->work_vt)) != CE_OK) return rc;
+        if (build_ref) {
+            CE_LAUNCH_ON(ctx, s1, "ssim2_ref_hblur_L1-5", h_tail_ref, dim3(tab.blk_end[tab.n - 1], 3, n_refs_used), dim3(HB_THREADS), 0,
+                         (const float *)nullptr, b->d_pair_ref, (float *)nullptr, 0u, 0u, 0u, (size_t)0, b->max_refs, rg, tab,
+                         (const uint2 *)nullptr, (const uint32_t *)b->d_pair_first);
+            CE_LAUNCH_ON(ctx, s1, "ssim2_ref_vblur_L1-5", k_ssim2_ref_vblur<-1>, dim3(tab_v.blk_end[tab_v.n - 1], 3, n_refs_used), dim3(64), 0,
+                         (const float *)nullptr, (float *)nullptr, 0u, 0u, 0u, (size_t)0, rg, tab_v, ref_h, ref_blur);
+        }
         CE_LAUNCH_ON(ctx, s1, "ssim2_hblur_L1-5", h_tail, dim3(b->work_ht.len), dim3(HB_THREADS), 0,
                      (const float *)nullptr, b->d_pair_ref, (float *)nullptr, 0u, 0u, 0u, (size_t)0, b->max_refs, rg, tab,
                      (const uint2 *)b->work_ht.d, (const uint32_t *)b->d_pair_first);
 #define CE_VBLUR_TAIL_ARGS                                                                                                  \
     (const float *)nullptr, (const float *)nullptr, b->d_pair_ref, b->d_partials, 0u, 0u, 0u, (size_t)0, b->max_refs, 0u,        \
-        b->max_vblocks, rg, tab_v, (const uint2 *)b->work_vt.d, (const uint32_t *)b->d_pair_first, maps
-        if (store_maps)
+        b->max_vblocks, rg, tab_v, (const uint2 *)b->work_vt.d, (const uint32_t *)b->d_pair_first, maps, ref_blur
+        if (split && store_maps)
+            CE_LAUNCH_ON(ctx, s1, "ssim2_vblur_ssim_map_L1-5", vr_tail_map, dim3(b->work_vt.len), dim3(64), 0, CE_VBLUR_TAIL_ARGS);
+        else if (split)
+            CE_LAUNCH_ON(ctx, s1, "ssim2_vblur_ssim_L1-5", vr_tail, dim3(b->work_vt.len), dim3(64), 0, CE_VBLUR_TAIL_ARGS);
+        else if (store_maps)
             CE_LAUNCH_ON(ctx, s1, "ssim2_vblur_ssim_map_L1-5", v_tail_map, dim3(b->work_vt.len), dim3(64), 0, CE_VBLUR_TAIL_ARGS);
         else
             CE_LAUNCH_ON(ctx, s1, "ssim2_vblur_ssim_L1-5", v_tail, dim3(b->work_vt.len), dim3(64), 0, CE_VBLUR_TAIL_ARGS);
@@ -846,6 +974,7 @@
               b->d_scores, (uint32_t)levels, b->max_vblocks, g);
     CE_HIP(ctx, hipGetLastError());
     if (!cached) b->refs.built(CE_REF_SSIM2, d_refs, n_refs_used, (uint64_t)levels);
+    if (build_ref) b->refs.built(CE_REF_SSIM2_BLUR, d_refs, n_refs_used, (uint64_t)levels);
     return CE_OK;
 }
 
```

Result: faster. 21380 (median of 6 runs) (+1.5%).
